# nglaze00/SCoNe_GCN

Measured on NVIDIA B200. Metric: SCoNe train trajectories/sec, higher is better.
Workload: dtype f32

## Files before the change

include/scone_b200.h:

```cpp
#ifndef SCONE_B200_H
#define SCONE_B200_H

#include <stdint.h>

#ifdef __cplusplus
extern "C" {
#endif

#define SCONE_B200_VERSION 100

typedef struct scone_complex scone_complex;
typedef struct scone_model scone_model;

enum { SCONE_MODEL_SCONE = 0, SCONE_MODEL_EBLI = 1, SCONE_MODEL_BUNCH = 2 };
enum { SCONE_ACT_TANH = 0, SCONE_ACT_LEAKY_RELU = 1, SCONE_ACT_RELU = 2 };

int scone_version(void);
const char* scone_last_error(void);

int scone_complex_create(int32_t n_nodes, int32_t n_edges, int32_t n_tris,
                         const int32_t* edge_nodes , const int8_t* edge_signs ,
                         const int32_t* tri_edges , const int8_t* tri_signs ,
                         int32_t model, scone_complex** out);
int scone_complex_create_index_only(int32_t n_nodes, int32_t n_edges, int32_t n_tris,
                                    const int32_t* edge_nodes, const int8_t* edge_signs,
                                    const int32_t* tri_edges, const int8_t* tri_signs,
                                    int32_t model, scone_complex** out);
int scone_complex_destroy(scone_complex* cx);
int scone_complex_dims(const scone_complex* cx, int32_t* n_nodes, int32_t* n_edges, int32_t* n_tris,
                       int32_t* max_degree, int64_t* nnz0, int64_t* nnz1);
int scone_complex_get_shift_csr(const scone_complex* cx, int32_t which, int32_t* rowptr ,
                                int32_t* col , float* val );
int scone_complex_get_nbrhoods(const scone_complex* cx, int32_t* nbrhoods );
int scone_complex_get_edge_rank(const scone_complex* cx, int32_t* rank );


int scone_flows_to_dense(const scone_complex* cx, int32_t b, const int32_t* traj_ptr_dev ,
                         const int32_t* flow_edge_dev, const float* flow_val_dev, float* X_dev ,
                         uint8_t* occ_X_dev , void* stream);

int64_t scone_occ_scratch_bytes(const scone_complex* cx, int32_t b);
int scone_layer_forward(const scone_complex* cx, int32_t act, int32_t b, int32_t cin, int32_t cout,
                        const float* Hin_dev, const float* W0_dev, const float* W1_dev, const float* W2_dev,
                        float* Hout_dev, const uint8_t* occ_in_dev, uint8_t* occ_out_dev, uint8_t* occ_scratch_dev,
                        void* stream);

int64_t scone_layer_backward_workspace_bytes(int32_t cin, int32_t cout);
int scone_layer_backward(const scone_complex* cx, int32_t act, int32_t b, int32_t cin, int32_t cout,
                         const float* G_dev, const float* Hin_dev,
                         const float* W0_dev, const float* W1_dev, const float* W2_dev,
                         float* Gprev_dev, float* dW_dev, int32_t accumulate, void* workspace_dev,
                         const uint8_t* occ_g_dev, const uint8_t* occ_hin_dev, uint8_t* occ_gprev_dev,
                         uint8_t* occ_scratch_dev, void* stream);

int64_t scone_readout_workspace(int32_t b, int32_t C);
int scone_readout(const scone_complex* cx, int32_t act, int32_t b, int32_t C,
                  const float* HL_dev, const float* wout_dev, const int32_t* last_nodes_dev,
                  float* logprobs_dev,
                  const int32_t* target_idx_dev, const float* mask_dev, float scale,
                  float* GL_dev, float* dwout_dev, float* nll_sum_dev, float* count_dev, int32_t accumulate,
                  void* workspace_dev, const uint8_t* occ_HL_dev, uint8_t* occ_GL_dev, void* stream);

int scone_model_create(const scone_complex* cx, int32_t n_layers, const int32_t* hidden, int32_t micro_batch,
                       scone_model** out);
int scone_model_destroy(scone_model* m);
int64_t scone_model_num_params(const scone_model* m);
int scone_model_set_zero_fill(scone_model* m, int32_t on);
int scone_model_get_zero_fill(const scone_model* m);
int scone_model_set_pipeline(scone_model* m, int32_t which);
int scone_model_get_pipeline(const scone_model* m);
int scone_model_set_weights(scone_model* m, const float* weights_host);
int scone_model_get_weights(const scone_model* m, float* weights_host);
float* scone_model_weights_dev(scone_model* m);
float* scone_model_grads_dev(scone_model* m);

int scone_model_forward_host(scone_model* m, int32_t B, const int32_t* traj_ptr ,
                             const int32_t* flow_edge, const float* flow_val, const int32_t* last_nodes,
                             float* logprobs_out , void* stream);
int scone_model_forward_dev(scone_model* m, int32_t B, const int32_t* traj_ptr_dev, const int32_t* flow_edge_dev,
                            const float* flow_val_dev, const int32_t* last_nodes_dev, float* logprobs_dev, void* stream);

int scone_model_loss_grad_dev(scone_model* m, int32_t B, const int32_t* traj_ptr_dev, const int32_t* flow_edge_dev,
                              const float* flow_val_dev, const int32_t* last_nodes_dev,
                              const int32_t* target_idx_dev, const float* mask_dev, int32_t zero_first, void* stream);
int scone_model_loss_grad_host(scone_model* m, int32_t B, const int32_t* traj_ptr, const int32_t* flow_edge,
                               const float* flow_val, const int32_t* last_nodes,
                               const int32_t* target_idx, const float* mask, int32_t zero_first, void* stream);
int scone_accuracy_dev(int32_t B, int32_t D, const float* logprobs_dev, const int32_t* n_nbrs_dev,
                       const int32_t* target_idx_dev, const float* mask_dev, int32_t* out_dev , void* stream);
int scone_model_accuracy_host(scone_model* m, int32_t B, const int32_t* traj_ptr, const int32_t* flow_edge,
                              const float* flow_val, const int32_t* last_nodes, const int32_t* n_nbrs,
                              const int32_t* target_idx, const float* mask, int32_t* out_host , void* stream);
int scone_model_eval_host(scone_model* m, int32_t B, const int32_t* traj_ptr, const int32_t* flow_edge, const float* flow_val,
                          const int32_t* last_nodes, const int32_t* n_nbrs, const int32_t* target_idx, const float* mask,
                          int32_t* choice_out, int32_t* acc_out, float* nll_out, void* stream);
int scone_model_two_target_host(scone_model* m, int32_t B, const int32_t* true_idx, const int32_t* rand_idx, int32_t* out ,
                                void* stream);
int scone_model_read_grads(scone_model* m, float* out_host, void* stream);
int scone_model_read_grads_async(scone_model* m, float* out_pinned, void* stream);

int scone_model_adam_step(scone_model* m, int32_t step, float lr, float weight_decay, void* stream);

typedef struct scone_dp scone_dp;
int scone_dp_create(int32_t rank, int32_t world, int64_t n_floats, scone_dp** out);
int32_t scone_dp_handle_bytes(void);
int scone_dp_get_handle(scone_dp* dp, void* handle_out);
int scone_dp_open(scone_dp* dp, const void* handles_rank_major);
int scone_model_dp_adam_step(scone_model* m, scone_dp* dp, int32_t step, float lr, float wd, void* stream);
int scone_dp_status(scone_dp* dp, void* stream);
void scone_dp_destroy(scone_dp* dp);
int scone_model_plan_host(scone_model* m, int32_t B, const int32_t* traj_ptr, const int32_t* flow_edge, const float* flow_val,
                          const int32_t* last_nodes, void* stream);
int scone_model_plan_dev(scone_model* m, int32_t B, const int32_t* traj_ptr_dev, const int32_t* flow_edge_dev, const float* flow_val_dev,
                         const int32_t* last_nodes_dev, void* stream);
int scone_model_loss_grad_planned_host(scone_model* m, int32_t n, const int32_t* rows, const int32_t* target_idx, const float* mask,
                                       int32_t zero_first, void* stream);
int scone_model_loss_grad_planned_dev(scone_model* m, int32_t n, const int32_t* rows_dev, const int32_t* target_idx_dev, const float* mask_dev,
                                      int32_t zero_first, void* stream);
int scone_model_forward_planned_host(scone_model* m, int32_t n, const int32_t* rows, float* logprobs_out , void* stream);
int scone_model_check_overflow(scone_model* m, void* stream);
int scone_model_set_weights_keep_state(scone_model* m, const float* weights_host, void* stream);
int scone_model_fused_info(const scone_model* m, int32_t* out );
int scone_model_fused_read(scone_model* m, int32_t t, int32_t* hdr_out , uint32_t off, int32_t words, uint32_t* arena_out);
int scone_model_read_rows_done(scone_model* m, int64_t* out );

typedef struct scone_csr scone_csr;
typedef struct scone_bunch scone_bunch;
int scone_csr_create(int32_t rows, int32_t cols, const int32_t* rowptr , const int32_t* col, const float* val,
                     scone_csr** out);
int scone_csr_destroy(scone_csr* S);
int scone_bunch_create(const scone_csr* const* S7, int32_t n_nodes, int32_t n_edges, int32_t n_tris, int32_t max_degree,
                       const int32_t* nbrhoods , int32_t n_hidden, const int32_t* hidden,
                       int32_t micro_batch, scone_bunch** out);
int scone_bunch_destroy(scone_bunch* m);
int64_t scone_bunch_num_params(const scone_bunch* m);
float* scone_bunch_grads_dev(scone_bunch* m);
int scone_bunch_set_weights(scone_bunch* m, const float* weights_host, int32_t reset_adam);
int scone_bunch_get_weights(const scone_bunch* m, float* weights_host);
int scone_bunch_forward_host(scone_bunch* m, int32_t B, const int32_t* traj_ptr, const int32_t* flow_edge, const float* flow_val,
                             const int32_t* last_nodes, float* logprobs_out , void* stream);
int scone_bunch_loss_grad_host(scone_bunch* m, int32_t B, const int32_t* traj_ptr, const int32_t* flow_edge, const float* flow_val,
                               const int32_t* last_nodes, const int32_t* target_idx, const float* mask, int32_t zero_first,
                               void* stream);
int scone_bunch_read_grads(scone_bunch* m, float* out_host, void* stream);
int scone_bunch_adam_step(scone_bunch* m, int32_t step, float lr, float weight_decay, void* stream);

int scone_set_zero_fill(int32_t on);
int scone_get_zero_fill(void);

int scone_set_dense_kernel(int32_t which);
int scone_umma_status(void* stream);
int scone_set_dense_chunk(int32_t tiles);
int scone_get_dense_kernel(void);

int scone_profile_enable(int32_t on);
int scone_profile_reset(void);
int scone_profile_read(int32_t kind, int64_t* launches, double* total_ms);
int scone_profile_read_rows(int32_t kind, int64_t* rows);

int64_t scone_launch_count(void);

#ifdef __cplusplus
}
#endif
#endif
```

scone_gcn_b200/_lib.py:

```python
import ctypes as C
import os

_HERE = os.path.dirname(os.path.abspath(__file__))
_LIB = None


class LibraryMissing(RuntimeError):
    pass


class SconeError(RuntimeError):
    pass


def library_path():
    return os.path.join(_HERE, 'libscone_b200.so')


_i32, _i64, _f32, _vp = C.c_int32, C.c_int64, C.c_float, C.c_void_p
DEFAULT_DENSE_KERNEL = 3

SIGNATURES = {
    'scone_version': (C.c_int, []),
    'scone_last_error': (C.c_char_p, []),
    'scone_launch_count': (_i64, []),
    'scone_profile_enable': (C.c_int, [_i32]),
    'scone_profile_reset': (C.c_int, []),
    'scone_profile_read': (C.c_int, [_i32, C.POINTER(_i64), C.POINTER(C.c_double)]),
    'scone_profile_read_rows': (C.c_int, [_i32, C.POINTER(_i64)]),
    'scone_complex_create': (C.c_int, [_i32, _i32, _i32, _vp, _vp, _vp, _vp, _i32, C.POINTER(_vp)]),
    'scone_complex_create_index_only': (C.c_int, [_i32, _i32, _i32, _vp, _vp, _vp, _vp, _i32, C.POINTER(_vp)]),
    'scone_complex_destroy': (C.c_int, [_vp]),
    'scone_complex_dims': (C.c_int, [_vp] + [C.POINTER(_i32)] * 4 + [C.POINTER(_i64)] * 2),
    'scone_complex_get_shift_csr': (C.c_int, [_vp, _i32, _vp, _vp, _vp]),
    'scone_complex_get_nbrhoods': (C.c_int, [_vp, _vp]),
    'scone_complex_get_edge_rank': (C.c_int, [_vp, _vp]),
    'scone_flows_to_dense': (C.c_int, [_vp, _i32, _vp, _vp, _vp, _vp, _vp, _vp]),
    'scone_occ_scratch_bytes': (_i64, [_vp, _i32]),
    'scone_layer_forward': (C.c_int, [_vp, _i32, _i32, _i32, _i32, _vp, _vp, _vp, _vp, _vp, _vp, _vp, _vp, _vp]),
    'scone_layer_backward_workspace_bytes': (_i64, [_i32, _i32]),
    'scone_layer_backward': (C.c_int, [_vp, _i32, _i32, _i32, _i32, _vp, _vp, _vp, _vp, _vp, _vp, _vp, _i32, _vp, _vp, _vp, _vp, _vp, _vp]),
    'scone_readout_workspace': (_i64, [_i32, _i32]),
    'scone_readout': (C.c_int, [_vp, _i32, _i32, _i32, _vp, _vp, _vp, _vp, _vp, _vp, _f32, _vp, _vp, _vp, _vp, _i32, _vp, _vp, _vp, _vp]),
    'scone_set_zero_fill': (C.c_int, [_i32]),
    'scone_get_zero_fill': (C.c_int, []),
    'scone_set_dense_kernel': (C.c_int, [_i32]),
    'scone_set_dense_chunk': (C.c_int, [_i32]),
    'scone_get_dense_kernel': (C.c_int, []),
    'scone_umma_status': (C.c_int, [_vp]),
    'scone_csr_create': (C.c_int, [_i32, _i32, _vp, _vp, _vp, C.POINTER(_vp)]),
    'scone_csr_destroy': (C.c_int, [_vp]),
    'scone_bunch_create': (C.c_int, [_vp, _i32, _i32, _i32, _i32, _vp, _i32, _vp, _i32, C.POINTER(_vp)]),
    'scone_bunch_destroy': (C.c_int, [_vp]),
    'scone_bunch_num_params': (_i64, [_vp]),
    'scone_bunch_grads_dev': (_vp, [_vp]),
    'scone_bunch_set_weights': (C.c_int, [_vp, _vp, _i32]),
    'scone_bunch_get_weights': (C.c_int, [_vp, _vp]),
    'scone_bunch_forward_host': (C.c_int, [_vp, _i32, _vp, _vp, _vp, _vp, _vp, _vp]),
    'scone_bunch_loss_grad_host': (C.c_int, [_vp, _i32, _vp, _vp, _vp, _vp, _vp, _vp, _i32, _vp]),
    'scone_bunch_read_grads': (C.c_int, [_vp, _vp, _vp]),
    'scone_bunch_adam_step': (C.c_int, [_vp, _i32, _f32, _f32, _vp]),
    'scone_model_create': (C.c_int, [_vp, _i32, _vp, _i32, C.POINTER(_vp)]),
    'scone_model_destroy': (C.c_int, [_vp]),
    'scone_model_num_params': (_i64, [_vp]),
    'scone_model_set_zero_fill': (C.c_int, [_vp, _i32]),
    'scone_model_get_zero_fill': (C.c_int, [_vp]),
    'scone_model_set_pipeline': (C.c_int, [_vp, _i32]),
    'scone_model_get_pipeline': (C.c_int, [_vp]),
    'scone_model_set_weights': (C.c_int, [_vp, _vp]),
    'scone_model_get_weights': (C.c_int, [_vp, _vp]),
    'scone_model_weights_dev': (_vp, [_vp]),
    'scone_model_grads_dev': (_vp, [_vp]),
    'scone_model_forward_host': (C.c_int, [_vp, _i32, _vp, _vp, _vp, _vp, _vp, _vp]),
    'scone_model_forward_dev': (C.c_int, [_vp, _i32, _vp, _vp, _vp, _vp, _vp, _vp]),
    'scone_model_loss_grad_dev': (C.c_int, [_vp, _i32, _vp, _vp, _vp, _vp, _vp, _vp, _i32, _vp]),
    'scone_model_loss_grad_host': (C.c_int, [_vp, _i32, _vp, _vp, _vp, _vp, _vp, _vp, _i32, _vp]),
    'scone_accuracy_dev': (C.c_int, [_i32, _i32, _vp, _vp, _vp, _vp, _vp, _vp]),
    'scone_model_accuracy_host': (C.c_int, [_vp, _i32, _vp, _vp, _vp, _vp, _vp, _vp, _vp, _vp, _vp]),
    'scone_model_read_grads': (C.c_int, [_vp, _vp, _vp]),
    'scone_model_read_grads_async': (C.c_int, [_vp, _vp, _vp]),
    'scone_model_eval_host': (C.c_int, [_vp, _i32] + [_vp] * 10 + [_vp]),
    'scone_model_two_target_host': (C.c_int, [_vp, _i32, _vp, _vp, _vp, _vp]),
    'scone_model_adam_step': (C.c_int, [_vp, _i32, _f32, _f32, _vp]),
    'scone_dp_create': (C.c_int, [_i32, _i32, _i64, C.POINTER(_vp)]),
    'scone_dp_handle_bytes': (_i32, []),
    'scone_dp_get_handle': (C.c_int, [_vp, _vp]),
    'scone_dp_open': (C.c_int, [_vp, _vp]),
    'scone_model_dp_adam_step': (C.c_int, [_vp, _vp, _i32, _f32, _f32, _vp]),
    'scone_dp_status': (C.c_int, [_vp, _vp]),
    'scone_dp_destroy': (None, [_vp]),
    'scone_model_check_overflow': (C.c_int, [_vp, _vp]),
    'scone_model_plan_host': (C.c_int, [_vp, _i32, _vp, _vp, _vp, _vp, _vp]),
    'scone_model_plan_dev': (C.c_int, [_vp, _i32, _vp, _vp, _vp, _vp, _vp]),
    'scone_model_loss_grad_planned_host': (C.c_int, [_vp, _i32, _vp, _vp, _vp, _i32, _vp]),
    'scone_model_loss_grad_planned_dev': (C.c_int, [_vp, _i32, _vp, _vp, _vp, _i32, _vp]),
    'scone_model_forward_planned_host': (C.c_int, [_vp, _i32, _vp, _vp, _vp]),
    'scone_model_set_weights_keep_state': (C.c_int, [_vp, _vp, _vp]),
    'scone_model_fused_info': (C.c_int, [_vp, _vp]),
    'scone_model_fused_read': (C.c_int, [_vp, _i32, _vp, C.c_uint32, _i32, _vp]),
    'scone_model_read_rows_done': (C.c_int, [_vp, _vp]),
}


def lib():
    global _LIB
    if _LIB is not None:
        return _LIB
    path = library_path()
    if not os.path.exists(path):
        raise LibraryMissing(
            '%s not found: build it with `python __graft_entry__.py build` (or `make`). '
            'scone_gcn_b200 has no CPU fallback.' % path)
    L = C.CDLL(path)
    for name, (res, args) in SIGNATURES.items():
        f = getattr(L, name)
        f.restype, f.argtypes = res, args
    _LIB = L
    return L


def check(rc, what=''):
    if rc != 0:
        msg = lib().scone_last_error().decode('utf-8', 'replace')
        raise SconeError('%s failed (code %d): %s' % (what or 'scone call', rc, msg))


def ptr(a):
    if a is None:
        return None
    assert a.flags['C_CONTIGUOUS']
    return a.ctypes.data_as(C.c_void_p)


def dptr(t):
    if t is None:
        return None
    if isinstance(t, int):
        return C.c_void_p(t)
    assert t.is_cuda and t.is_contiguous()
    return C.c_void_p(t.data_ptr())
```

scone_gcn_b200/csrc/fused.cuh:

```cuda
#pragma once
#include "common.cuh"

constexpr int kFusedMaxL = 3;
constexpr int kFusedHdrW = 16;
constexpr int kFusedFlagOverflow = 1;
constexpr int kFusedFlagRetry = 2;

struct PlanArgs {
    const int32_t* traj_ptr;
    const int32_t* flow_edge;
    const float* flow_val;
    const int32_t* last_nodes;
    const int32_t* rank;
    const int32_t* nbrhoods;
    const int32_t* inc_ptr;
    const int2* inc_ent;
    const int32_t* mptr;
    const int2* ment;
    int N, D, E, L;
    int HS, hshift;
    const unsigned* cone_ptr;
    const uint32_t* cone_ent;
    int LV;
    int EC;
    int M;
    const unsigned long long* node_off;
    const unsigned* tb_rowptr;
    const int2* tb_ent;
    const unsigned* pair_ptr;
    const int2* tb_pairs;
    const int* pair_off;
    int* hdr;
    uint32_t* arena;
    unsigned long long* bump;
    unsigned long long arena_words;
    int* overflow;
    int tier;
    int n_work;
    int t0;
    const int* n_in;
    const int* in_list;
    int* n_retry;
    int* retry;
};

#ifdef __CUDACC__
template <int THREADS>
__device__ inline int fused_block_scan_excl(int* a, int n, int* s_warp) {
    const int tid = threadIdx.x, lane = tid & 31, warp = tid >> 5;
    const int per = (n + THREADS - 1) / THREADS;
    const int lo = min(n, tid * per), hi = min(n, lo + per);
    int sum = 0;
    for (int i = lo; i < hi; ++i) sum += a[i];
    int inc = sum;
#pragma unroll
    for (int o = 1; o < 32; o <<= 1) {
        const int v = __shfl_up_sync(0xffffffffu, inc, o);
        if (lane >= o) inc += v;
    }
    __syncthreads();
    if (lane == 31) s_warp[warp] = inc;
    __syncthreads();
    int base = 0, total = 0;
#pragma unroll
    for (int w = 0; w < THREADS / 32; ++w) {
        const int v = s_warp[w];
        if (w < warp) base += v;
        total += v;
    }
    int run = base + inc - sum;
    for (int i = lo; i < hi; ++i) {
        const int v = a[i];
        a[i] = run;
        run += v;
    }
    if (tid == 0) a[n] = total;
    __syncthreads();
    return total;
}
#endif

struct FusedState {
    int L = 0, C = 0;
    int64_t n_params = 0;
    int bound_cone = 0, bound_list = 0;
    unsigned* d_cone_ptr = nullptr;
    uint32_t* d_cone_ent = nullptr;
    unsigned long long cone_entries = 0;
    bool tb_rows = false;
    unsigned long long* d_node_off = nullptr;
    unsigned* d_tb_rowptr = nullptr;
    int2* d_tb_ent = nullptr;
    unsigned* d_pair_ptr = nullptr;
    int2* d_tb_pairs = nullptr;
    int* d_pair_off = nullptr;
    unsigned long long tb_entries = 0, tb_bytes = 0;
    int tbM0 = 0, tbLV0 = 0, tbM1 = 0, tbLV1 = 0, tbM = 0, tbLV = 0;
    size_t tb_smem0 = 0, tb_smem1 = 0, tb_smem = 0;
    bool tb_two_tiers = false, tb_mid_tier = false;
    int quantile_cone = 0;
    int HS = 0, LV = 0, EC = 0, hshift = 0;
    int HS0 = 0, LV0 = 0, EC0 = 0, hshift0 = 0;
    bool two_tiers = false;
    int flow_room = 0;
    size_t plan_smem0 = 0;
    unsigned long long worst_words = 0;
    int* d_retry = nullptr;
    size_t plan_smem = 0, traj_smem_small = 0, traj_smem_big = 0;
    int cap_rows = 0, big_rows = 0, grid_small = 0, grid_big = 0, chunk = 0;
    size_t scratch_stride = 0;
    unsigned long long arena_words = 0;
    int* d_hdr = nullptr;
    uint32_t* d_arena = nullptr;
    unsigned long long* d_bump = nullptr;
    float* d_partial = nullptr;
    float* d_scratch = nullptr;
    int* d_stats = nullptr;
    unsigned long long* d_rows_done = nullptr;
    uint32_t* d_sort = nullptr;
    void* d_sort_tmp = nullptr;
    size_t sort_tmp_bytes = 0;
    int sort_cap = 0;
    int* d_set_hdr = nullptr;
    uint32_t* d_set_arena = nullptr;
    unsigned long long* d_set_bump = nullptr;
    unsigned long long set_arena_words = 0;
    int set_cap = 0, set_n = 0;
};

int scone_table_build(const scone_complex* cx, FusedState* f, int L, bool* ok);
int scone_table_plan_launch(const FusedState* f, PlanArgs p, int b, int num_sms, cudaStream_t st, int phase = 2);
void scone_table_destroy(FusedState* f);

bool scone_fused_supported(const scone_complex* cx, int n_layers, const int32_t* hidden);
int scone_fused_create(const scone_complex* cx, int L, int C, int mb, int64_t n_params, FusedState** out);
void scone_fused_destroy(FusedState* f);
int scone_fused_run(const scone_complex* cx, FusedState* f, int act, int b, const int32_t* traj_ptr, const int32_t* flow_edge,
                    const float* flow_val, const int32_t* last_nodes, const float* W, const int64_t* w_off, float* logprobs,
                    const int32_t* target_idx, const float* mask, float* grad, int* overflow, bool count_rows, cudaStream_t st);
int scone_fused_begin(FusedState* f, cudaStream_t st);
int scone_fused_plan_part(const scone_complex* cx, FusedState* f, int off, int b, const int32_t* traj_ptr, const int32_t* flow_edge,
                          const float* flow_val, const int32_t* last_nodes, int* overflow, cudaStream_t st,
                          bool defer_tiers = false);
int scone_fused_plan_finish(const scone_complex* cx, FusedState* f, int B, const int32_t* traj_ptr, const int32_t* flow_edge,
                            const float* flow_val, const int32_t* last_nodes, int* overflow, cudaStream_t st);
int scone_fused_compute(const scone_complex* cx, FusedState* f, int act, int b, const float* W, const int64_t* w_off, float* logprobs,
                        const int32_t* target_idx, const float* mask, float* grad, bool count_rows, cudaStream_t st);
int scone_fused_plan_set(const scone_complex* cx, FusedState* f, int B, const int32_t* traj_ptr, const int32_t* flow_edge,
                         const float* flow_val, const int32_t* last_nodes, int* overflow, cudaStream_t st);
int scone_fused_run_planned(const scone_complex* cx, FusedState* f, int act, int n, const int32_t* rows_dev, const float* W, const int64_t* w_off,
                            float* logprobs, const int32_t* target_idx, const float* mask, float* grad, bool count_rows, cudaStream_t st);
int scone_fused_last_retries(FusedState* f);
int scone_fused_read(FusedState* f, int t, int* hdr_out, unsigned off, int words, uint32_t* arena_out);
```

scone_gcn_b200/csrc/scone_fused.cu:

```cuda
#include <algorithm>
#include <cstdlib>
#include <cub/device/device_radix_sort.cuh>
#include "common.cuh"
#include "fused.cuh"

namespace {

#include "slab_common.cuh"

constexpr int kTrajThreads = 256;
constexpr int kFuMaxD = 128;
constexpr uint32_t kNoRow = 0xFFFFu;
constexpr uint32_t kFlaggedKey = 0xFFFFFFu;

template <int ACT>
__device__ __forceinline__ float fu_act(float z) {
    if (ACT == SCONE_ACT_TANH) return scone_tanh(z);
    if (ACT == SCONE_ACT_LEAKY_RELU) return z >= 0.f ? z : 0.01f * z;
    return fmaxf(z, 0.f);
}
template <int ACT>
__device__ __forceinline__ float fu_dact(float h) {
    if (ACT == SCONE_ACT_TANH) return 1.f - h * h;
    if (ACT == SCONE_ACT_LEAKY_RELU) return h >= 0.f ? 1.f : 0.01f;
// ... 825 lines not shown
                }
                fu_dw<C>(acc[l - 2], hprev + (size_t)r0 * G::LDH, tile, nr);
                __syncthreads();
                fu_product<C, true>(tile, Wl, nr, [&](int r, int col, float v0, float v1) {
                    const float2 hv = *reinterpret_cast<const float2*>(hprev + (size_t)(r0 + r) * G::LDH + col);
                    *reinterpret_cast<float2*>(gprev + (size_t)(r0 + r) * G::LDH + col) =
                        make_float2(v0 * fu_dact<ACT>(hv.x), v1 * fu_dact<ACT>(hv.y));
                });
                cp_async_wait_all();
                __syncthreads();
                r0 += nr;
            }
            if (np_ == 0) {
                cp_async_wait_all();
                __syncthreads();
            }
            pf = pf_next;
        }
        if (tid < 3 * C) {
            const int k = tid / C, c = tid % C;
            const float* g1 = rows;
            float s = acc1;
            for (int r = 0; r < n[1]; ++r) s = fmaf(l1[3 * r + k], g1[(size_t)r * G::LDH + c], s);
            acc1 = s;
        }
        if (have_next && !issued_next) {
            cp_async_wait_all();
            __syncthreads();
            pf_first_next = issue_first(s_hdr[(k + 1) & 1], l1s + ((k + 1) & 1) * G::SL1);
        }
        pf_first = pf_first_next;
        t = t_next;
        have = have_next;
    }

    if (a.rows_done != nullptr && tid == 0 && (n_fwd | n_bwd)) {
        atomicAdd(a.rows_done, n_fwd);
        atomicAdd(a.rows_done + 1, n_bwd);
    }
    if (!GRAD) return;
    float* P = a.partial + (size_t)blockIdx.x * (a.n_params + 2);
    if (tid < 3 * C) P[a.w_off[tid / C] + tid % C] = acc1;
    {
        const int g = lane >> 2, tig = lane & 3;
        const int mt = warp % G::NMT, ntg = warp / G::NMT;
#pragma unroll
        for (int l = 2; l <= kFusedMaxL; ++l) {
            if (l > L) break;
#pragma unroll
            for (int s = 0; s < G::TPW; ++s) {
                const int nt = ntg + G::WPM * s;
                if (nt >= G::NNT) continue;
                const int nn = 8 * nt + 2 * tig, term = nn / C, co = nn % C;
                float* dst = P + a.w_off[3 * (l - 1) + term];
                const int ci = 16 * mt + g;
                dst[ci * C + co] = acc[l - 2][s][0];
                dst[ci * C + co + 1] = acc[l - 2][s][1];
                dst[(ci + 8) * C + co] = acc[l - 2][s][2];
                dst[(ci + 8) * C + co + 1] = acc[l - 2][s][3];
            }
        }
    }
    if (tid < C) P[a.w_off[3 * L] + tid] = acc_out;
    if (warp == 0) {
        float s = acc_nll;
#pragma unroll
        for (int o = 16; o > 0; o >>= 1) s += __shfl_xor_sync(0xffffffffu, s, o);
        if (lane == 0) {
            P[a.n_params] = s;
            P[a.n_params + 1] = acc_cnt;
        }
    }
}

__global__ void __launch_bounds__(256) fused_cost_kernel(const int* __restrict__ hdr, const int32_t* __restrict__ rows, int b, int L,
                                                         uint32_t* __restrict__ keys, int32_t* __restrict__ vals) {
    const int t = blockIdx.x * blockDim.x + threadIdx.x;
    if (t >= b) return;
    const int* h = hdr + (size_t)(rows != nullptr ? rows[t] : t) * kFusedHdrW;
    int tot = 0;
    for (int l = 1; l <= L; ++l) tot += h[l];
    keys[t] = h[0] != 0 ? kFlaggedKey : min((uint32_t)tot, kFlaggedKey - 1u);
    vals[t] = t;
}

__global__ void __launch_bounds__(256) fused_reduce_kernel(const float* __restrict__ partial, int nparts, int n, float* __restrict__ out) {
    __shared__ float red[8][32];
    const int lane = threadIdx.x & 31, warp = threadIdx.x >> 5;
    const int i = blockIdx.x * 32 + lane;
    float s = 0.f;
    if (i < n)
        for (int p = warp; p < nparts; p += 8) s += partial[(size_t)p * n + i];
    red[warp][lane] = s;
    __syncthreads();
    if (warp == 0 && i < n)
        out[i] += ((red[0][lane] + red[1][lane]) + (red[2][lane] + red[3][lane])) + ((red[4][lane] + red[5][lane]) + (red[6][lane] + red[7][lane]));
}

size_t plan_smem_bytes(int HS, int LV, int EC) {
    return (size_t)HS * 18 + (size_t)(LV + 4) * 8 + (size_t)LV * 10 + (size_t)EC * 2 + 16;
}

template <int C>
size_t traj_smem_bytes(int D, int cap_rows) {
    using G = FuGeom<C>;
    size_t fl = (size_t)(kFusedMaxL - 1) * 3 * C * G::LDW + 3 * C + C + (size_t)G::CH * G::LDA + (size_t)D * C + 2 * ((D + 3) & ~3) +
                2 * (size_t)G::SE + G::SP + 2 * G::SL1 + (size_t)cap_rows * G::LDH;
    return fl * sizeof(float);
}

template <int C, int ACT, bool GRAD>
int launch_traj(const TrajArgs& base, int grid_small, int grid_big, size_t smem_small, size_t smem_big, cudaStream_t st) {
    static bool configured = false;
    if (!configured) {
        SCONE_CUDA(cudaFuncSetAttribute(fused_traj_kernel<C, ACT, GRAD, false>, cudaFuncAttributeMaxDynamicSharedMemorySize, 227 * 1024 - 1024));
        SCONE_CUDA(cudaFuncSetAttribute(fused_traj_kernel<C, ACT, GRAD, true>, cudaFuncAttributeMaxDynamicSharedMemorySize, 227 * 1024 - 1024));
        configured = true;
    }
    TrajArgs a = base;
    fused_traj_kernel<C, ACT, GRAD, false><<<grid_small, kTrajThreads, smem_small, st>>>(a);
    SCONE_LAUNCHED();
    if (grid_big > 0) {
        if (GRAD) a.partial = base.partial + (size_t)grid_small * (base.n_params + 2);
        fused_traj_kernel<C, ACT, GRAD, true><<<grid_big, kTrajThreads, smem_big, st>>>(a);
        SCONE_LAUNCHED();
    }
    return 0;
}

template <int C, bool GRAD>
int dispatch_traj(int act, const TrajArgs& a, int gs, int gb, size_t ss, size_t sb, cudaStream_t st) {
    switch (act) {
        case SCONE_ACT_TANH: return launch_traj<C, SCONE_ACT_TANH, GRAD>(a, gs, gb, ss, sb, st);
        case SCONE_ACT_LEAKY_RELU: return launch_traj<C, SCONE_ACT_LEAKY_RELU, GRAD>(a, gs, gb, ss, sb, st);
        case SCONE_ACT_RELU: return launch_traj<C, SCONE_ACT_RELU, GRAD>(a, gs, gb, ss, sb, st);
    }
    scone_set_error("unknown activation %d", act);
    return 2;
}

int run_traj(FusedState* f, int act, TrajArgs& t, float* grad, cudaStream_t st) {
    const bool want_grad = grad != nullptr;
    const int n = t.b;
    if (n > f->sort_cap) {
        cudaFree(f->d_sort);
        cudaFree(f->d_sort_tmp);
        f->d_sort = nullptr;
        f->d_sort_tmp = nullptr;
        f->sort_cap = 0;
        uint32_t* k = nullptr;
        int32_t* v = nullptr;
        size_t bytes = 0;
        SCONE_CUDA(cub::DeviceRadixSort::SortPairsDescending(nullptr, bytes, k, k, v, v, n, 0, 24, st));
        SCONE_CUDA(cudaMalloc((void**)&f->d_sort, 4 * (size_t)n * sizeof(uint32_t)));
        SCONE_CUDA(cudaMalloc((void**)&f->d_sort_tmp, bytes ? bytes : 16));
        f->sort_tmp_bytes = bytes;
        f->sort_cap = n;
    }
    uint32_t* k_in = f->d_sort;
    uint32_t* k_out = k_in + f->sort_cap;
    int32_t* v_in = reinterpret_cast<int32_t*>(k_out + f->sort_cap);
    int32_t* v_out = v_in + f->sort_cap;
    ScopedProf prof(want_grad ? SCONE_K_LAYER_BWD : SCONE_K_LAYER_FWD, st);
    fused_cost_kernel<<<(n + 255) / 256, 256, 0, st>>>(t.hdr, t.rows, n, f->L, k_in, v_in);
    SCONE_LAUNCHED();
    size_t bytes = f->sort_tmp_bytes;
    SCONE_CUDA(cub::DeviceRadixSort::SortPairsDescending(f->d_sort_tmp, bytes, k_in, k_out, v_in, v_out, n, 0, 24, st));
    t.okeys = k_out;
    t.order = v_out;
    int rc;
    if (f->C == 32)
        rc = want_grad ? dispatch_traj<32, true>(act, t, f->grid_small, f->grid_big, f->traj_smem_small, f->traj_smem_big, st)
                       : dispatch_traj<32, false>(act, t, f->grid_small, f->grid_big, f->traj_smem_small, f->traj_smem_big, st);
    else
        rc = want_grad ? dispatch_traj<16, true>(act, t, f->grid_small, f->grid_big, f->traj_smem_small, f->traj_smem_big, st)
                       : dispatch_traj<16, false>(act, t, f->grid_small, f->grid_big, f->traj_smem_small, f->traj_smem_big, st);
    if (rc) return rc;
    if (want_grad) {
        const int np = (int)f->n_params + 2;
        fused_reduce_kernel<<<(np + 31) / 32, 256, 0, st>>>(f->d_partial, f->grid_small + f->grid_big, np, grad);
        SCONE_LAUNCHED();
    }
    return 0;
}

}

bool scone_fused_supported(const scone_complex* cx, int n_layers, const int32_t* hidden) {
    if (cx->d_mptr == nullptr || cx->D > kFuMaxD || cx->D < 1 || n_layers < 1 || n_layers > kFusedMaxL) return false;
    for (int l = 0; l < n_layers; ++l)
        if (hidden[l] != hidden[0] || (hidden[l] != 16 && hidden[l] != 32)) return false;
    return true;
}

void scone_fused_destroy(FusedState* f) {
    if (!f) return;
    cudaFree(f->d_hdr); cudaFree(f->d_retry); cudaFree(f->d_arena); cudaFree(f->d_set_hdr); cudaFree(f->d_set_arena); cudaFree(f->d_set_bump); cudaFree(f->d_bump); cudaFree(f->d_partial); cudaFree(f->d_scratch); cudaFree(f->d_stats);
    cudaFree(f->d_rows_done); cudaFree(f->d_sort); cudaFree(f->d_sort_tmp);
    scone_table_destroy(f);
    delete f;
}

static void table_shape(int entries, int* HS, int* hshift) {
    int hs = 256;
    while (hs * 3 / 4 < entries + 1) hs *= 2;
    *HS = hs;
    *hshift = 32;
    for (int v = hs; v > 1; v >>= 1) --*hshift;
}

int scone_fused_create(const scone_complex* cx, int L, int C, int mb, int64_t n_params, FusedState** out) {
    *out = nullptr;
    if ((unsigned)cx->E >= (1u << 30)) return 0;
    FusedState* f = new FusedState();
    f->L = L;
    f->C = C;
    f->n_params = n_params;
    {
        bool ok = false;
        const int rc = scone_table_build(cx, f, L, &ok);
        if (rc || !ok) {
            scone_fused_destroy(f);
            return rc;
        }
    }
    int max_row = 1;
    {
        std::vector<int32_t> mp((size_t)cx->E + 1);
        SCONE_CUDA(cudaMemcpy(mp.data(), cx->d_mptr, mp.size() * sizeof(int32_t), cudaMemcpyDeviceToHost));
        for (int e = 0; e < cx->E; ++e) max_row = std::max(max_row, mp[e + 1] - mp[e]);
    }
    constexpr int kMaxPlanSmem = 225 * 1024;
    f->LV = (f->bound_list + 63) & ~63;
    table_shape(f->bound_cone, &f->HS, &f->hshift);
    f->EC = (int)std::min<long long>((long long)f->bound_list * max_row, 1ll << 30);
    f->EC = (f->EC + 63) & ~63;
    {
        const size_t fixed = plan_smem_bytes(f->HS, f->LV, 0);
        if (fixed + 2 * (size_t)f->EC > (size_t)kMaxPlanSmem && fixed + 2 * 8192 <= (size_t)kMaxPlanSmem)
            f->EC = (int)(((size_t)kMaxPlanSmem - fixed) / 2) & ~63;
    }
    f->plan_smem = plan_smem_bytes(f->HS, f->LV, f->EC);
    if (!f->tb_rows && (f->plan_smem > (size_t)kMaxPlanSmem || f->bound_list >= 0xFFFF || f->HS > 32768)) {
        scone_fused_destroy(f);
        return 0;
    }
    {
        table_shape(f->quantile_cone, &f->HS0, &f->hshift0);
        f->LV0 = std::min(192, f->LV);
        f->EC0 = std::min(3072, f->EC);
        f->two_tiers = f->HS0 < f->HS || f->LV0 < f->LV || f->EC0 < f->EC;
        if (!f->two_tiers) {
            f->HS0 = f->HS;
            f->hshift0 = f->hshift;
        }
        auto env_int = [](const char* name, int dflt) {
            const char* v = getenv(name);
            return v && *v ? atoi(v) : dflt;
        };
        if (f->two_tiers) {
            const int hs0 = env_int("SCONE_FUSED_HS0", f->HS0);
            if (hs0 != f->HS0 && hs0 >= 256 && hs0 <= f->HS && (hs0 & (hs0 - 1)) == 0) table_shape((hs0 * 3) / 4 - 1, &f->HS0, &f->hshift0);
            f->LV0 = std::min(env_int("SCONE_FUSED_LV0", f->LV0), f->LV);
            f->EC0 = std::min(env_int("SCONE_FUSED_EC0", f->EC0), f->EC);
        }
        f->plan_smem0 = plan_smem_bytes(f->HS0, f->LV0, f->EC0);
    }
    SCONE_CUDA(cudaFuncSetAttribute(fused_plan_kernel<256>, cudaFuncAttributeMaxDynamicSharedMemorySize, kMaxPlanSmem));
    SCONE_CUDA(cudaFuncSetAttribute(fused_plan_kernel<1024>, cudaFuncAttributeMaxDynamicSharedMemorySize, kMaxPlanSmem));
    const int ldh = C + 8;
    f->cap_rows = C == 32 ? 192 : 384;
    f->big_rows = L * f->bound_list;
    f->traj_smem_small = C == 32 ? traj_smem_bytes<32>(cx->D, f->cap_rows) : traj_smem_bytes<16>(cx->D, f->cap_rows);
    f->traj_smem_big = C == 32 ? traj_smem_bytes<32>(cx->D, 0) : traj_smem_bytes<16>(cx->D, 0);
    if (f->traj_smem_small > 113 * 1024) {
        const size_t over = f->traj_smem_small - 113 * 1024;
        const int less = (int)((over + ldh * 4 - 1) / (ldh * 4));
        f->cap_rows = f->cap_rows > less + 32 ? f->cap_rows - less : 32;
        f->traj_smem_small = C == 32 ? traj_smem_bytes<32>(cx->D, f->cap_rows) : traj_smem_bytes<16>(cx->D, f->cap_rows);
    }
    f->grid_small = 2 * cx->num_sms;
    f->grid_big = f->big_rows > f->cap_rows ? 2 * cx->num_sms : 0;
    if (f->grid_big) {
        f->scratch_stride = (size_t)f->big_rows * ldh;
        SCONE_CUDA(cudaMalloc((void**)&f->d_scratch, (size_t)f->grid_big * f->scratch_stride * sizeof(float)));
    }
    SCONE_CUDA(cudaMalloc((void**)&f->d_partial, (size_t)(f->grid_small + f->grid_big) * (n_params + 2) * sizeof(float)));
    const unsigned long long bl = (unsigned long long)f->bound_list;
    unsigned long long worst = 3 * bl + 2 + (unsigned long long)(cx->D + 3) + 2ull * cx->D * cx->D + 16;
    for (int l = 2; l <= L; ++l)
        worst += 2 * (bl + 3) + 4 * bl * (unsigned long long)max_row;
    const unsigned long long budget_words = (1ull << 30) - 1024;
    const unsigned long long share_words = 16 * 1024;
    f->worst_words = worst;
    if (worst * (unsigned long long)mb <= budget_words) {
        f->chunk = mb;
        f->arena_words = worst * (unsigned long long)mb;
    } else {
        f->chunk = (int)std::min<unsigned long long>((unsigned long long)mb, std::max<unsigned long long>(1, budget_words / std::min(worst, share_words)));
        f->arena_words = std::min(budget_words, worst * (unsigned long long)f->chunk);
    }
    SCONE_CUDA(cudaMalloc((void**)&f->d_arena, f->arena_words * sizeof(uint32_t)));
    SCONE_CUDA(cudaMalloc((void**)&f->d_hdr, (size_t)f->chunk * kFusedHdrW * sizeof(int)));
    SCONE_CUDA(cudaMalloc((void**)&f->d_retry, 2 * (size_t)f->chunk * sizeof(int)));
    SCONE_CUDA(cudaMalloc((void**)&f->d_bump, 2 * sizeof(unsigned long long)));
    SCONE_CUDA(cudaMalloc((void**)&f->d_rows_done, 4 * sizeof(unsigned long long)));
    SCONE_CUDA(cudaMemset(f->d_rows_done, 0, 4 * sizeof(unsigned long long)));
    *out = f;
    return 0;
}

static int launch_plans(const scone_complex* cx, const FusedState* f, PlanArgs p, int b, cudaStream_t st) {
    if (f->tb_rows) return scone_table_plan_launch(f, p, b, cx->num_sms, st);
    p.tier = 0; p.n_work = b;
    p.HS = f->HS0; p.LV = f->LV0; p.EC = f->EC0; p.hshift = f->hshift0;
    int* retry = p.retry;
    if (!f->two_tiers) p.retry = nullptr;
    fused_plan_kernel<256><<<b, 256, f->plan_smem0, st>>>(p);
    SCONE_LAUNCHED();
    if (f->two_tiers) {
        p.tier = 1; p.HS = f->HS; p.LV = f->LV; p.EC = f->EC; p.hshift = f->hshift; p.n_in = p.n_retry; p.in_list = retry; p.retry = nullptr;
        fused_plan_kernel<1024><<<std::min(b, cx->num_sms), 1024, f->plan_smem, st>>>(p);
        SCONE_LAUNCHED();
    }
    return 0;
}

int scone_fused_begin(FusedState* f, cudaStream_t st) {
    SCONE_CUDA(cudaMemsetAsync(f->d_bump, 0, 2 * sizeof(unsigned long long), st));
    return 0;
}

static PlanArgs plan_args(const scone_complex* cx, FusedState* f, int off, const int32_t* traj_ptr, const int32_t* flow_edge,
                          const float* flow_val, const int32_t* last_nodes, int* overflow) {
    PlanArgs p{};
    p.traj_ptr = traj_ptr + off; p.flow_edge = flow_edge; p.flow_val = flow_val; p.last_nodes = last_nodes + off;
    p.rank = cx->d_rank; p.nbrhoods = cx->d_nbrhoods; p.inc_ptr = cx->d_inc_ptr; p.inc_ent = cx->d_inc_ent;
    p.mptr = cx->d_mptr; p.ment = cx->d_ment; p.cone_ptr = f->d_cone_ptr; p.cone_ent = f->d_cone_ent;
    p.N = cx->N; p.D = cx->D; p.E = cx->E; p.L = f->L;
    p.hdr = f->d_hdr + (size_t)off * kFusedHdrW; p.arena = f->d_arena; p.bump = f->d_bump; p.arena_words = f->arena_words; p.overflow = overflow;
    p.n_retry = reinterpret_cast<int*>(f->d_bump + 1); p.retry = f->d_retry;
    return p;
}

int scone_fused_plan_part(const scone_complex* cx, FusedState* f, int off, int b, const int32_t* traj_ptr, const int32_t* flow_edge,
                          const float* flow_val, const int32_t* last_nodes, int* overflow, cudaStream_t st, bool defer_tiers) {
    if (b <= 0) return 0;
    SCONE_REQUIRE(off >= 0 && off + b <= f->chunk, "scone_fused_plan_part: trajectories %d .. %d exceed the planned chunk of %d", off, off + b, f->chunk);
    ScopedProf prof(SCONE_K_CONE, st);
    if (defer_tiers && f->tb_rows) {
        PlanArgs p = plan_args(cx, f, 0, traj_ptr, flow_edge, flow_val, last_nodes, overflow);
        p.t0 = off;
        return scone_table_plan_launch(f, p, b, cx->num_sms, st, 0);
    }
    if (off > 0) SCONE_CUDA(cudaMemsetAsync(f->d_bump + 1, 0, sizeof(unsigned long long), st));
    return launch_plans(cx, f, plan_args(cx, f, off, traj_ptr, flow_edge, flow_val, last_nodes, overflow), b, st);
}

int scone_fused_plan_finish(const scone_complex* cx, FusedState* f, int B, const int32_t* traj_ptr, const int32_t* flow_edge,
                            const float* flow_val, const int32_t* last_nodes, int* overflow, cudaStream_t st) {
    if (B <= 0 || !f->tb_rows) return 0;
    ScopedProf prof(SCONE_K_CONE, st);
    return scone_table_plan_launch(f, plan_args(cx, f, 0, traj_ptr, flow_edge, flow_val, last_nodes, overflow), B, cx->num_sms, st, 1);
}

int scone_fused_compute(const scone_complex* cx, FusedState* f, int act, int b, const float* W, const int64_t* w_off, float* logprobs,
                        const int32_t* target_idx, const float* mask, float* grad, bool count_rows, cudaStream_t st) {
    if (b <= 0) return 0;
    TrajArgs t;
    t.hdr = f->d_hdr; t.arena = f->d_arena; t.rows = nullptr; t.W = W;
    for (int i = 0; i <= 3 * kFusedMaxL; ++i) t.w_off[i] = i <= 3 * f->L ? (int)w_off[i] : 0;
    t.L = f->L; t.b = b; t.D = cx->D; t.n_params = (int)f->n_params;
    t.logprobs = logprobs; t.target_idx = target_idx; t.mask = mask;
    t.partial = f->d_partial; t.scratch = f->d_scratch; t.scratch_stride = f->scratch_stride;
    t.cap_rows = f->cap_rows; t.big_rows = f->big_rows;
    t.rows_done = count_rows ? f->d_rows_done : nullptr;
    return run_traj(f, act, t, grad, st);
}

int scone_fused_run(const scone_complex* cx, FusedState* f, int act, int b, const int32_t* traj_ptr, const int32_t* flow_edge,
                    const float* flow_val, const int32_t* last_nodes, const float* W, const int64_t* w_off, float* logprobs,
                    const int32_t* target_idx, const float* mask, float* grad, int* overflow, bool count_rows, cudaStream_t st) {
    if (b <= 0) return 0;
    SCONE_REQUIRE(b <= f->chunk, "scone_fused_run: chunk of %d trajectories exceeds the planned %d", b, f->chunk);
    int rc = scone_fused_begin(f, st);
    if (!rc) rc = scone_fused_plan_part(cx, f, 0, b, traj_ptr, flow_edge, flow_val, last_nodes, overflow, st);
    if (!rc) rc = scone_fused_compute(cx, f, act, b, W, w_off, logprobs, target_idx, mask, grad, count_rows, st);
    return rc;
}

int scone_fused_plan_set(const scone_complex* cx, FusedState* f, int B, const int32_t* traj_ptr, const int32_t* flow_edge,
                         const float* flow_val, const int32_t* last_nodes, int* overflow, cudaStream_t st) {
    if (B > f->set_cap) {
        cudaFree(f->d_set_hdr);
        cudaFree(f->d_set_arena);
        f->d_set_hdr = nullptr;
        f->d_set_arena = nullptr;
        f->set_cap = 0;
        const unsigned long long budget_words = (1ull << 30) - 1024;
        f->set_arena_words = std::min(budget_words, f->worst_words * (unsigned long long)B);
        SCONE_CUDA(cudaMalloc((void**)&f->d_set_hdr, (size_t)B * kFusedHdrW * sizeof(int)));
        SCONE_CUDA(cudaMalloc((void**)&f->d_set_arena, f->set_arena_words * sizeof(uint32_t)));
        if (!f->d_set_bump) SCONE_CUDA(cudaMalloc((void**)&f->d_set_bump, 2 * sizeof(unsigned long long)));
        f->set_cap = B;
    }
    f->set_n = 0;
    SCONE_CUDA(cudaMemsetAsync(f->d_set_bump, 0, 2 * sizeof(unsigned long long), st));
    PlanArgs p{};
    p.flow_edge = flow_edge; p.flow_val = flow_val;
    p.rank = cx->d_rank; p.nbrhoods = cx->d_nbrhoods; p.inc_ptr = cx->d_inc_ptr; p.inc_ent = cx->d_inc_ent;
    p.mptr = cx->d_mptr; p.ment = cx->d_ment; p.cone_ptr = f->d_cone_ptr; p.cone_ent = f->d_cone_ent;
    p.N = cx->N; p.D = cx->D; p.E = cx->E; p.L = f->L;
    p.arena = f->d_set_arena; p.bump = f->d_set_bump; p.arena_words = f->set_arena_words; p.overflow = overflow;
    p.n_retry = reinterpret_cast<int*>(f->d_set_bump + 1); p.retry = f->d_retry;
    ScopedProf prof(SCONE_K_CONE, st);
    for (int off = 0; off < B; off += f->chunk) {
        const int b = std::min(f->chunk, B - off);
        SCONE_CUDA(cudaMemsetAsync(f->d_set_bump + 1, 0, sizeof(unsigned long long), st));
        p.traj_ptr = traj_ptr + off; p.last_nodes = last_nodes + off; p.hdr = f->d_set_hdr + (size_t)off * kFusedHdrW;
        const int rc = launch_plans(cx, f, p, b, st);
        if (rc) return rc;
    }
    f->set_n = B;
    return 0;
}

int scone_fused_run_planned(const scone_complex* cx, FusedState* f, int act, int n, const int32_t* rows_dev, const float* W, const int64_t* w_off,
                            float* logprobs, const int32_t* target_idx, const float* mask, float* grad, bool count_rows, cudaStream_t st) {
    if (n <= 0) return 0;
    SCONE_REQUIRE(f->set_n > 0, "scone_fused_run_planned: no planned set (call scone_model_plan_* first)");
    SCONE_REQUIRE(rows_dev != nullptr || n <= f->set_n, "scone_fused_run_planned: %d trajectories requested, the planned set holds %d", n, f->set_n);
    TrajArgs t;
    t.hdr = f->d_set_hdr; t.arena = f->d_set_arena; t.rows = rows_dev; t.W = W;
    for (int i = 0; i <= 3 * kFusedMaxL; ++i) t.w_off[i] = i <= 3 * f->L ? (int)w_off[i] : 0;
    t.L = f->L; t.b = n; t.D = cx->D; t.n_params = (int)f->n_params;
    t.logprobs = logprobs; t.target_idx = target_idx; t.mask = mask;
    t.partial = f->d_partial; t.scratch = f->d_scratch; t.scratch_stride = f->scratch_stride;
    t.cap_rows = f->cap_rows; t.big_rows = f->big_rows;
    t.rows_done = count_rows ? f->d_rows_done : nullptr;
    return run_traj(f, act, t, grad, st);
}

int scone_fused_last_retries(FusedState* f) {
    unsigned long long v[2] = {0, 0};
    if (cudaDeviceSynchronize() != cudaSuccess) return -1;
    if (cudaMemcpy(v, f->d_bump, sizeof(v), cudaMemcpyDeviceToHost) != cudaSuccess) return -1;
    return (int)(v[1] & 0xffffffffull);
}

int scone_fused_read(FusedState* f, int t, int* hdr_out, unsigned off, int words, uint32_t* arena_out) {
    SCONE_CUDA(cudaDeviceSynchronize());
    if (hdr_out) SCONE_CUDA(cudaMemcpy(hdr_out, f->d_hdr + (size_t)t * kFusedHdrW, kFusedHdrW * sizeof(int), cudaMemcpyDeviceToHost));
    if (arena_out && words > 0) SCONE_CUDA(cudaMemcpy(arena_out, f->d_arena + off, (size_t)words * sizeof(uint32_t), cudaMemcpyDeviceToHost));
    return 0;
}
```

scone_gcn_b200/csrc/scone_model.cu:

```cuda
#include <algorithm>
#include <cstring>
#include "common.cuh"
#include "fused.cuh"

struct scone_model {
    const scone_complex* cx = nullptr;
    int32_t L = 0, mb = 0, act = 0, cmax = 0;
    std::vector<int32_t> hidden;
    std::vector<int64_t> w_off;
    int64_t n_params = 0;
    float *d_w = nullptr, *d_m = nullptr, *d_v = nullptr, *d_grad = nullptr;
    float* d_X = nullptr;
    std::vector<float*> d_H;
    std::vector<float*> d_G;
    std::vector<uint8_t*> d_occH;
    std::vector<uint8_t*> d_occG;
    cudaStream_t side = nullptr;
    cudaStream_t compute = nullptr;
    cudaEvent_t ev_fork = nullptr, ev_join = nullptr;
    cudaEvent_t ev_begin = nullptr;
    cudaStream_t copy = nullptr;
    cudaEvent_t ev_copy0 = nullptr, ev_part[8] = {nullptr, nullptr, nullptr, nullptr, nullptr, nullptr, nullptr, nullptr};
    cudaEvent_t ev_plan_done = nullptr;
    long long staging_epoch = 0, plan_done_epoch = -1;
// ... 357 lines not shown
        const int cout = m->hidden[l];
        ScopedProf prof(l == 0 ? SCONE_K_LAYER0_FWD : SCONE_K_LAYER_FWD, s);
        const float *W0 = m->d_w + m->w_off[3 * l], *W1 = m->d_w + m->w_off[3 * l + 1], *W2 = m->d_w + m->w_off[3 * l + 2];
        int rc;
        if (l == 0)
            rc = scone_rows_layer0_forward(cx, m->act, b, cout, m->d_X, W0, W1, W2, m->d_cH[0], m->d_rowsC[0], cone_n(m, 0), nullptr,
                                           m->row_cap, m->d_overflow, s);
        else
            rc = scone_slab_forward_rows(cx, m->act, b, cin, cout, m->d_cH[l - 1], W0, W1, W2, m->d_cH[l], nullptr, m->d_rowsC[l],
                                         cone_n(m, l), scone_prof_row_counter(SCONE_K_LAYER_FWD), m->d_bmGr[l - 1], m->d_prefG[l - 1],
                                         m->row_cap, m->d_overflow, s);
        if (rc) return rc;
        cin = cout;
    }
    return 0;
}

int cone_readout(scone_model* m, int32_t b, const int32_t* last, float* logprobs, bool grad, const int32_t* tgt, const float* mask,
                 cudaStream_t s) {
    const scone_complex* cx = m->cx;
    const int L = m->L, CL = m->hidden[L - 1];
    const float* wout = m->d_w + m->w_off[3 * L];
    ScopedProf prof(SCONE_K_READOUT, s);
    if (scone_rows_readout_forward(cx, b, CL, m->d_cH[L - 1], wout, last, logprobs, m->d_bmGr[L - 1], m->d_prefG[L - 1], nullptr, nullptr, s))
        return 1;
    if (!grad) return 0;
    return scone_rows_readout_backward(cx, m->act, b, CL, m->d_cH[L - 1], wout, last, logprobs, tgt, mask, 1.f, m->d_cG[L - 1],
                                       cone_n(m, L - 1), m->row_cap, m->d_overflow, m->d_grad + m->w_off[3 * L], m->d_grad + m->n_params,
                                       m->d_grad + m->n_params + 1, 1, (float*)m->d_ws, m->d_bmGr[L - 1], m->d_prefG[L - 1],
                                       m->d_bmGr[L - 1], m->d_prefG[L - 1], s);
}

int cone_backward_mb(scone_model* m, int32_t b, cudaStream_t s) {
    const scone_complex* cx = m->cx;
    const int L = m->L;
    const int a_cap = m->row_cap < m->a_cap ? m->row_cap : m->a_cap;
    SCONE_CUDA(cudaMemset2DAsync(m->d_nrows + 1, 2 * sizeof(int), 0, sizeof(int), (size_t)(L + 1), s));
    for (int l = L - 1; l >= 1; --l) {
        ScopedProf prof(SCONE_K_LAYER_BWD, s);
        int rc = scone_rows_backward(cx, m->act, b, m->hidden[l - 1], m->hidden[l], m->d_cG[l], m->d_cH[l - 1], m->d_cG[l - 1], m->d_Abuf,
                                     m->d_w + m->w_off[3 * l], m->d_w + m->w_off[3 * l + 1], m->d_w + m->w_off[3 * l + 2], m->d_rowsC[l - 1],
                                     cone_n(m, l - 1), m->d_bmGr[l], m->d_bmGr[l - 1], a_cap, m->d_overflow, m->d_grad + m->w_off[3 * l], 1,
                                     (float*)m->d_ws, m->d_prefG[l], m->d_prefG[l - 1], true, s);
        if (rc) return rc;
    }
    ScopedProf prof(SCONE_K_LAYER0_BWD, s);
    return scone_rows_layer0_backward(cx, b, m->hidden[0], m->d_X, m->d_cG[0], m->d_rowsC[0], cone_n(m, 0), m->d_grad + m->w_off[0], 1,
                                      (float*)m->d_ws, m->row_cap, s);
}

}

extern "C" int scone_model_create(const scone_complex* cx, int32_t n_layers, const int32_t* hidden, int32_t micro_batch,
                                  scone_model** out) {
    SCONE_REQUIRE(out != nullptr, "scone_model_create: out is NULL");
    *out = nullptr;
    SCONE_REQUIRE(cx && hidden && n_layers >= 1 && micro_batch >= 1, "scone_model_create: bad arguments");
    SCONE_REQUIRE(!cx->host_only, "scone_model_create: index-only complex has no device arrays");
    scone_model* m = new scone_model();
    m->cx = cx;
    m->L = n_layers;
    m->mb = micro_batch;
    m->act = cx->model == SCONE_MODEL_EBLI ? SCONE_ACT_LEAKY_RELU : SCONE_ACT_TANH;
    m->hidden.assign(hidden, hidden + n_layers);
    int64_t off = 0;
    int cin = 1;
    for (int l = 0; l < n_layers; ++l) {
        const int c = hidden[l];
        if (!(c == 8 || c == 16 || c == 32 || c == 64)) {
            scone_set_error("scone_model_create: hidden width %d of layer %d unsupported (8, 16, 32 or 64)", c, l);
            delete m;
            return 2;
        }
        if (l > 0 && !(c == cin || c == 2 * cin || 2 * c == cin)) {
            scone_set_error("scone_model_create: consecutive widths %d -> %d unsupported (ratio must be 1/2, 1 or 2)", cin, c);
            delete m;
            return 2;
        }
        for (int k = 0; k < 3; ++k) {
            m->w_off.push_back(off);
            off += (int64_t)cin * c;
        }
        m->cmax = c > m->cmax ? c : m->cmax;
        cin = c;
    }
    m->w_off.push_back(off);
    off += cin;
    m->n_params = off;
    const size_t E = cx->E, mb = micro_batch;
    int rc = 0;
    auto alloc = [&](void** p, size_t bytes) {
        if (rc) return;
        cudaError_t e = cudaMalloc(p, bytes ? bytes : 4);
        if (e != cudaSuccess) {
            scone_set_error("scone_model_create: cudaMalloc(%zu bytes) failed: %s", bytes, cudaGetErrorString(e));
            rc = 1;
        }
    };
    alloc((void**)&m->d_w, off * sizeof(float));
    alloc((void**)&m->d_m, off * sizeof(float));
    alloc((void**)&m->d_v, off * sizeof(float));
    alloc((void**)&m->d_grad, (off + 2) * sizeof(float));
    m->d_H.assign(n_layers, nullptr);
    m->d_G.assign(n_layers, nullptr);
    m->d_occH.assign(n_layers, nullptr);
    m->d_occG.assign(n_layers, nullptr);
    m->rows_ok = scone_rows_supported(cx, n_layers, hidden) && E * mb < ((size_t)1 << 32);
    m->pipeline = m->rows_ok ? ((cx->D <= 32 || E * mb >= ((size_t)1 << 31)) ? 3 : 2) : 0;
    if (scone_fused_supported(cx, n_layers, hidden)) {
        if (scone_fused_create(cx, n_layers, hidden[0], micro_batch, m->n_params, &m->fused)) {
            delete m;
            return 1;
        }
        if (m->fused) m->pipeline = 4;
    }
    if (m->pipeline != 4 && !m->rows_ok && E * mb >= ((size_t)1 << 31)) {
        scone_set_error("scone_model_create: E * micro_batch = %zu needs the row-list pipeline (widths 16 / 32, E * micro_batch < 2^32)", E * mb);
        delete m;
        return 2;
    }
    int64_t ws = scone_readout_workspace_bytes(micro_batch, m->cmax);
    if (scone_rows_dw_workspace_bytes(m->cmax, m->cmax) > ws) ws = scone_rows_dw_workspace_bytes(m->cmax, m->cmax);
    cin = 1;
    for (int l = 0; l < n_layers; ++l) {
        int64_t w = scone_layer_backward_workspace_bytes(cin, hidden[l]);
        ws = w > ws ? w : ws;
        cin = hidden[l];
    }
    alloc(&m->d_ws, ws);
    alloc((void**)&m->d_logp, mb * (size_t)(cx->D > 0 ? cx->D : 1) * sizeof(float));
    if (!rc) {
        int prio_lo = 0, prio_hi = 0;
        cudaDeviceGetStreamPriorityRange(&prio_lo, &prio_hi);
        cudaStreamCreateWithPriority(&m->side, cudaStreamNonBlocking, prio_lo);
        cudaStreamCreateWithPriority(&m->compute, cudaStreamNonBlocking, prio_hi);
        cudaEventCreateWithFlags(&m->ev_fork, cudaEventDisableTiming);
        cudaEventCreateWithFlags(&m->ev_join, cudaEventDisableTiming);
        cudaEventCreateWithFlags(&m->ev_begin, cudaEventDisableTiming);
        m->ev_fill.assign(2 * n_layers, nullptr);
        for (auto& e : m->ev_fill) cudaEventCreateWithFlags(&e, cudaEventDisableTiming);
        cudaMemset(m->d_w, 0, off * sizeof(float));
        cudaMemset(m->d_m, 0, off * sizeof(float));
        cudaMemset(m->d_v, 0, off * sizeof(float));
        cudaMemset(m->d_grad, 0, (off + 2) * sizeof(float));
    }
    if (!rc) rc = ensure_buffers(m);
    if (rc) {
        scone_model_destroy(m);
        return rc;
    }
    *out = m;
    return 0;
}

extern "C" int scone_model_destroy(scone_model* m) {
    if (!m) return 0;
    cudaFree(m->d_w); cudaFree(m->d_m); cudaFree(m->d_v); cudaFree(m->d_grad); cudaFree(m->d_X);
    for (float* p : m->d_H) cudaFree(p);
    for (uint8_t* p : m->d_occH) cudaFree(p);
    for (uint8_t* p : m->d_occG) cudaFree(p);
    cudaFree(m->d_occS); cudaFree(m->d_occX); cudaFree(m->d_bmX); cudaFree(m->d_bmG);
    for (uint32_t* p : m->d_bmH) cudaFree(p);
    for (uint32_t* p : m->d_bmGr) cudaFree(p);
    for (uint32_t* p : m->d_prefH) cudaFree(p);
    for (uint32_t* p : m->d_prefG) cudaFree(p);
    for (float* p : m->d_cH) cudaFree(p);
    for (float* p : m->d_cG) cudaFree(p);
    for (uint32_t* p : m->d_rowsC) cudaFree(p);
    for (uint32_t* p : m->d_bmC) cudaFree(p);
    cudaFree(m->d_rows); cudaFree(m->d_nrows); cudaFree(m->d_overflow); cudaFree(m->d_tickets); cudaFree(m->d_Abuf);
    for (float* p : m->d_G) cudaFree(p);
    cudaFree(m->d_ws); cudaFree(m->d_logp);
    scone_fused_destroy(m->fused);
    if (m->side) cudaStreamDestroy(m->side);
    if (m->compute) cudaStreamDestroy(m->compute);
    if (m->ev_fork) cudaEventDestroy(m->ev_fork);
    if (m->ev_join) cudaEventDestroy(m->ev_join);
    if (m->ev_begin) cudaEventDestroy(m->ev_begin);
    if (m->copy) cudaStreamDestroy(m->copy);
    if (m->ev_copy0) cudaEventDestroy(m->ev_copy0);
    if (m->ev_plan_done) cudaEventDestroy(m->ev_plan_done);
    for (auto e : m->ev_part) if (e) cudaEventDestroy(e);
    for (auto e : m->ev_fill) if (e) cudaEventDestroy(e);
    cudaFree(m->d_ptr); cudaFree(m->d_edge); cudaFree(m->d_last); cudaFree(m->d_tgt); cudaFree(m->d_val);
    cudaFree(m->d_mask); cudaFree(m->d_logp_all); cudaFree(m->d_nn); cudaFree(m->d_acc);
    cudaFree(m->d_choice); cudaFree(m->d_rand); cudaFree(m->d_evalf);
    delete m;
    return 0;
}

extern "C" int64_t scone_model_num_params(const scone_model* m) { return m ? m->n_params : -1; }
extern "C" int scone_model_set_zero_fill(scone_model* m, int32_t on) {
    SCONE_REQUIRE(m != nullptr, "scone_model_set_zero_fill: NULL model");
    SCONE_REQUIRE(!on || (size_t)m->cx->E * m->mb < ((size_t)1 << 31), "scone_model_set_zero_fill: E * micro_batch >= 2^31 runs on pipeline 3 only");
    m->zero_fill = on != 0;
    return ensure_buffers(m);
}
extern "C" int scone_model_get_zero_fill(const scone_model* m) { return m && m->zero_fill ? 1 : 0; }
extern "C" int scone_model_set_pipeline(scone_model* m, int32_t which) {
    SCONE_REQUIRE(m != nullptr && which >= 0 && which <= 4,
                  "scone_model_set_pipeline: 0 (unit kernels, byte flags), 1 (row lists, dense tensors), 2 (row lists, compact tensors), "
                  "3 (compact row lists over the readout cone) or 4 (trajectory-fused kernels)");
    SCONE_REQUIRE(which != 4 || m->fused != nullptr,
                  "scone_model_set_pipeline: the fused pipeline needs one uniform hidden width of 16 or 32, at most 3 layers, and cones that fit "
                  "its shared-memory tables");
    SCONE_REQUIRE(which == 0 || which == 4 || m->rows_ok, "scone_model_set_pipeline: the row-list pipelines need hidden widths in {16, 32}");
    SCONE_REQUIRE(which >= 3 || (size_t)m->cx->E * m->mb < ((size_t)1 << 31),
                  "scone_model_set_pipeline: E * micro_batch >= 2^31 runs on pipelines 3 / 4 only");
    SCONE_REQUIRE(which != 3 || (size_t)m->cx->E * m->mb < ((size_t)1 << 32), "scone_model_set_pipeline: pipeline 3 needs E * micro_batch < 2^32");
    const int old = m->pipeline;
    m->pipeline = which;
    if (ensure_buffers(m)) {
        m->pipeline = old;
        return 1;
    }
    return 0;
}
extern "C" int scone_model_get_pipeline(const scone_model* m) { return m ? (m->zero_fill ? 0 : m->pipeline) : -1; }
extern "C" float* scone_model_weights_dev(scone_model* m) { return m ? m->d_w : nullptr; }
extern "C" float* scone_model_grads_dev(scone_model* m) { return m ? m->d_grad : nullptr; }

extern "C" int scone_model_set_weights(scone_model* m, const float* w) {
    SCONE_REQUIRE(m && w, "scone_model_set_weights: NULL argument");
    SCONE_CUDA(cudaMemcpy(m->d_w, w, m->n_params * sizeof(float), cudaMemcpyHostToDevice));
    SCONE_CUDA(cudaMemset(m->d_m, 0, m->n_params * sizeof(float)));
    SCONE_CUDA(cudaMemset(m->d_v, 0, m->n_params * sizeof(float)));
    return 0;
}

extern "C" int scone_model_get_weights(const scone_model* m, float* w) {
    SCONE_REQUIRE(m && w, "scone_model_get_weights: NULL argument");
    SCONE_CUDA(cudaMemcpy(w, m->d_w, m->n_params * sizeof(float), cudaMemcpyDeviceToHost));
    return 0;
}

static int fork_to_compute(scone_model* m, void* user_st) {
    SCONE_CUDA(cudaEventRecord(m->ev_fork, as_stream(user_st)));
    SCONE_CUDA(cudaStreamWaitEvent(m->compute, m->ev_fork, 0));
    return 0;
}
static int join_from_compute(scone_model* m, void* user_st) {
    SCONE_CUDA(cudaEventRecord(m->ev_join, m->compute));
    SCONE_CUDA(cudaStreamWaitEvent(as_stream(user_st), m->ev_join, 0));
    return 0;
}

static int finish_call(scone_model* m, int rc, void* user_st) {
    if (rc) {
        m->x_clean = false;
        m->cone_clean = false;
    }
    const int jr = join_from_compute(m, user_st);
    return rc ? rc : jr;
}

static int fused_call(scone_model* m, int32_t B, const int32_t* ptr, const int32_t* edge, const float* val, const int32_t* last,
                      float* logprobs, const int32_t* tgt, const float* mask, bool grad, cudaStream_t s) {
    const int step = m->fused->chunk < m->mb ? m->fused->chunk : m->mb;
    for (int32_t off = 0; off < B; off += step) {
        const int32_t b = B - off < step ? B - off : step;
        int rc = scone_fused_run(m->cx, m->fused, m->act, b, ptr + off, edge, val, last + off, m->d_w, m->w_off.data(),
                                 logprobs ? logprobs + (size_t)off * m->cx->D : nullptr, grad ? tgt + off : nullptr,
                                 grad ? mask + off : nullptr, grad ? m->d_grad : nullptr, m->d_overflow, g_scone_prof, s);
        if (rc) return rc;
    }
    return 0;
}

static bool fused_host_overlap_ok(const scone_model* m, int32_t B, int64_t nnz) {
    const bool rows = m->pipeline >= 1 && !m->zero_fill;
    return rows && m->pipeline == 4 && m->fused && B >= 512 && B <= m->fused->chunk && B <= m->mb && nnz >= (1 << 13);
}

static int fused_host_overlapped(scone_model* m, int32_t B, const int32_t* ptr, const int32_t* edge, const float* val, float* logprobs_dev,
                                 bool grad, int32_t zero_first, cudaStream_t s) {
    constexpr int kMaxParts = 4;
    const int kParts = B >= 4 * 4096 ? 4 : (B >= 2 * 4096 ? 2 : 1);
    if (!m->copy) {
        SCONE_CUDA(cudaStreamCreateWithFlags(&m->copy, cudaStreamNonBlocking));
        SCONE_CUDA(cudaEventCreateWithFlags(&m->ev_copy0, cudaEventDisableTiming));
        SCONE_CUDA(cudaEventCreateWithFlags(&m->ev_plan_done, cudaEventDisableTiming));
        for (auto& e : m->ev_part) SCONE_CUDA(cudaEventCreateWithFlags(&e, cudaEventDisableTiming));
    }
    if (m->plan_done_epoch >= 0 && m->plan_done_epoch == m->staging_epoch - 1) {
        SCONE_CUDA(cudaStreamWaitEvent(m->copy, m->ev_plan_done, 0));
    } else {
        SCONE_CUDA(cudaEventRecord(m->ev_copy0, s));
        SCONE_CUDA(cudaStreamWaitEvent(m->copy, m->ev_copy0, 0));
    }
    int32_t b0[kMaxParts + 1];
    for (int k = 0; k <= kParts; ++k) b0[k] = (int32_t)((int64_t)B * k / kParts);
    for (int k = 0; k < kParts; ++k) {
        const int64_t q0 = ptr[b0[k]], q1 = ptr[b0[k + 1]];
        if (q1 > q0) {
            SCONE_CUDA(cudaMemcpyAsync(m->d_edge + q0, edge + q0, (q1 - q0) * sizeof(int32_t), cudaMemcpyHostToDevice, m->copy));
            SCONE_CUDA(cudaMemcpyAsync(m->d_val + q0, val + q0, (q1 - q0) * sizeof(float), cudaMemcpyHostToDevice, m->copy));
        }
        SCONE_CUDA(cudaEventRecord(m->ev_part[k], m->copy));
    }
    if (fork_to_compute(m, (void*)s)) return 1;
    cudaStream_t c = m->compute;
    if (grad && zero_first) SCONE_CUDA(cudaMemsetAsync(m->d_grad, 0, (m->n_params + 2) * sizeof(float), c));
    int rc = scone_fused_begin(m->fused, c);
    for (int k = 0; k < kParts && !rc; ++k) {
        SCONE_CUDA(cudaStreamWaitEvent(c, m->ev_part[k], 0));
        rc = scone_fused_plan_part(m->cx, m->fused, b0[k], b0[k + 1] - b0[k], m->d_ptr, m->d_edge, m->d_val, m->d_last, m->d_overflow, c,
                                   kParts > 1);
    }
    if (!rc && kParts > 1) rc = scone_fused_plan_finish(m->cx, m->fused, B, m->d_ptr, m->d_edge, m->d_val, m->d_last, m->d_overflow, c);
    if (!rc) {
        SCONE_CUDA(cudaEventRecord(m->ev_plan_done, c));
        m->plan_done_epoch = m->staging_epoch;
    } else {
        m->plan_done_epoch = -1;
    }
    if (!rc)
        rc = scone_fused_compute(m->cx, m->fused, m->act, B, m->d_w, m->w_off.data(), logprobs_dev, grad ? m->d_tgt : nullptr,
                                 grad ? m->d_mask : nullptr, grad ? m->d_grad : nullptr, g_scone_prof, c);
    return finish_call(m, rc, (void*)s);
}

extern "C" int scone_model_forward_dev(scone_model* m, int32_t B, const int32_t* ptr, const int32_t* edge, const float* val,
                                       const int32_t* last, float* logprobs, void* user_st) {
    SCONE_REQUIRE(m && ptr && last && logprobs && B >= 0, "scone_model_forward_dev: bad arguments");
    if (fork_to_compute(m, user_st)) return 1;
    void* st = (void*)m->compute;
    const scone_complex* cx = m->cx;
    const bool rows = m->pipeline >= 1 && !m->zero_fill;
    if (rows && m->pipeline == 4) return finish_call(m, fused_call(m, B, ptr, edge, val, last, logprobs, nullptr, nullptr, false, as_stream(st)), user_st);
    int rc = 0;
    for (int32_t off = 0; off < B && !rc; off += m->mb) {
        const int32_t b = B - off < m->mb ? B - off : m->mb;
        if (rows && m->pipeline == 3) {
            rc = cone_build_mb(m, b, ptr + off, edge, val, last + off, as_stream(st));
            if (!rc) rc = cone_forward_mb(m, b, as_stream(st));
            if (!rc) rc = cone_readout(m, b, last + off, logprobs + (size_t)off * cx->D, false, nullptr, nullptr, as_stream(st));
            if (!rc) rc = rows_clear_x(m, b, ptr + off, edge, val, as_stream(st));
            if (!rc) rc = cone_clear_mb(m, b, as_stream(st));
            continue;
        }
        if (rows) {
            rc = rows_forward_mb(m, b, ptr + off, edge, val, as_stream(st));
            if (!rc) rc = rows_readout(m, b, last + off, logprobs + (size_t)off * cx->D, false, nullptr, nullptr, as_stream(st));
            if (!rc) rc = rows_clear_x(m, b, ptr + off, edge, val, as_stream(st));
            continue;
        }
        m->x_clean = false;
        rc = start_fills(m, b, false, as_stream(st));
        if (!rc) rc = forward_mb(m, b, ptr + off, edge, val, st);
        if (!rc)
            rc = scone_readout_ws(cx, m->act, b, m->hidden[m->L - 1], m->d_H[m->L - 1], m->d_w + m->w_off[3 * m->L], last + off,
                                  logprobs + (size_t)off * cx->D, nullptr, nullptr, 0.f, nullptr, nullptr, nullptr, nullptr, 0,
                                  nullptr, m->d_occH[m->L - 1], nullptr, st);
    }
    return finish_call(m, rc, user_st);
}

extern "C" int scone_model_loss_grad_dev(scone_model* m, int32_t B, const int32_t* ptr, const int32_t* edge, const float* val,
                                         const int32_t* last, const int32_t* tgt, const float* mask, int32_t zero_first,
                                         void* user_st) {
    SCONE_REQUIRE(m && ptr && last && tgt && mask && B >= 0, "scone_model_loss_grad_dev: bad arguments");
    if (fork_to_compute(m, user_st)) return 1;
    void* st = (void*)m->compute;
    const scone_complex* cx = m->cx;
    const int L = m->L;
    cudaStream_t s = as_stream(st);
    if (zero_first) SCONE_CUDA(cudaMemsetAsync(m->d_grad, 0, (m->n_params + 2) * sizeof(float), s));
    const bool rows = m->pipeline >= 1 && !m->zero_fill;
    if (rows && m->pipeline == 4) return finish_call(m, fused_call(m, B, ptr, edge, val, last, nullptr, tgt, mask, true, s), user_st);
    int rc = 0;
    for (int32_t off = 0; off < B && !rc; off += m->mb) {
        const int32_t b = B - off < m->mb ? B - off : m->mb;
        if (rows && m->pipeline == 3) {
            rc = cone_build_mb(m, b, ptr + off, edge, val, last + off, s);
            if (!rc) rc = cone_forward_mb(m, b, s);
            if (!rc) rc = cone_readout(m, b, last + off, m->d_logp, true, tgt + off, mask + off, s);
            if (!rc) rc = cone_backward_mb(m, b, s);
            if (!rc) rc = rows_clear_x(m, b, ptr + off, edge, val, s);
            if (!rc) rc = cone_clear_mb(m, b, s);
            continue;
        }
        if (rows) {
            rc = rows_forward_mb(m, b, ptr + off, edge, val, s);
            if (!rc) rc = rows_readout(m, b, last + off, m->d_logp, true, tgt + off, mask + off, s);
            if (!rc) rc = rows_backward_mb(m, b, s);
            if (!rc) rc = rows_clear_x(m, b, ptr + off, edge, val, s);
            continue;
        }
        m->x_clean = false;
        rc = start_fills(m, b, true, s);
        if (!rc) rc = forward_mb(m, b, ptr + off, edge, val, st);
        const int CL = m->hidden[L - 1];
        if (!rc && wait_fill(m, L + (L - 1), s)) rc = 1;
        if (rc) break;
        g_scone_hints.out_bm = m->d_bmG;
        rc = scone_readout_ws(cx, m->act, b, CL, m->d_H[L - 1], m->d_w + m->w_off[3 * L], last + off, m->d_logp, tgt + off,
                              mask + off, 1.f, m->d_G[L - 1], m->d_grad + m->w_off[3 * L], m->d_grad + m->n_params,
                              m->d_grad + m->n_params + 1, 1, m->d_ws, m->d_occH[L - 1], m->d_occG[L - 1], st);
        int wl = -1, tt = 0;
        for (int l = L - 1; l >= 0 && !rc; --l) {
            const int cout = m->hidden[l], cin = l > 0 ? m->hidden[l - 1] : 1;
            const float* Hin = l > 0 ? m->d_H[l - 1] : m->d_X;
            if (l > 0 && wait_fill(m, L + (l - 1), s)) {
                rc = 1;
                break;
            }
            g_scone_hints.in_wl = wl;
            g_scone_hints.in_tt = tt;
            if (l == L - 1) g_scone_hints.in_bm = m->d_bmG;
            rc = scone_layer_backward(cx, m->act, b, cin, cout, m->d_G[l], Hin, m->d_w + m->w_off[3 * l],
                                      m->d_w + m->w_off[3 * l + 1], m->d_w + m->w_off[3 * l + 2], l > 0 ? m->d_G[l - 1] : nullptr,
                                      m->d_grad + m->w_off[3 * l], 1, m->d_ws, m->d_occG[l], l > 0 ? m->d_occH[l - 1] : nullptr,
                                      l > 0 ? m->d_occG[l - 1] : nullptr, m->d_occS, st);
            wl = g_scone_hints.out_wl;
            tt = g_scone_hints.out_tt;
        }
    }
    return finish_call(m, rc, user_st);
}

extern "C" int scone_model_forward_host(scone_model* m, int32_t B, const int32_t* ptr, const int32_t* edge, const float* val,
                                        const int32_t* last, float* logprobs_out, void* st) {
    SCONE_REQUIRE(m && ptr && last && logprobs_out && B >= 0, "scone_model_forward_host: bad arguments");
    if (B == 0) return 0;
    cudaStream_t s = as_stream(st);
    const int64_t nnz = ptr[B];
    int rc = ensure_staging(m, B, nnz);
    if (rc) return rc;
    SCONE_CUDA(cudaMemcpyAsync(m->d_ptr, ptr, (B + 1) * sizeof(int32_t), cudaMemcpyHostToDevice, s));
    SCONE_CUDA(cudaMemcpyAsync(m->d_last, last, B * sizeof(int32_t), cudaMemcpyHostToDevice, s));
    if (fused_host_overlap_ok(m, B, nnz)) {
        rc = fused_host_overlapped(m, B, ptr, edge, val, m->d_logp_all, false, 0, s);
    } else {
        SCONE_CUDA(cudaMemcpyAsync(m->d_edge, edge, nnz * sizeof(int32_t), cudaMemcpyHostToDevice, s));
        SCONE_CUDA(cudaMemcpyAsync(m->d_val, val, nnz * sizeof(float), cudaMemcpyHostToDevice, s));
        rc = scone_model_forward_dev(m, B, m->d_ptr, m->d_edge, m->d_val, m->d_last, m->d_logp_all, st);
    }
    if (rc) return rc;
    SCONE_CUDA(cudaMemcpyAsync(logprobs_out, m->d_logp_all, (size_t)B * m->cx->D * sizeof(float), cudaMemcpyDeviceToHost, s));
    int overflow = 0;
    if (m->d_overflow) SCONE_CUDA(cudaMemcpyAsync(&overflow, m->d_overflow, sizeof(int), cudaMemcpyDeviceToHost, s));
    SCONE_CUDA(cudaStreamSynchronize(s));
    if (overflow) {
        cudaMemset(m->d_overflow, 0, sizeof(int));
        m->cone_clean = false;
        scone_set_error("scone_model: a micro-batch exceeded a row-list capacity (%d rows per compact tensor, %d cone edges per trajectory "
                        "and layer); the log-probs are incomplete — use a smaller micro-batch or scone_model_set_pipeline(m, 2 / 0)",
                        m->row_cap, 2048);
        return 4;
    }
    return 0;
}

extern "C" int scone_accuracy_dev(int32_t B, int32_t D, const float* logprobs, const int32_t* n_nbrs, const int32_t* target_idx,
                                  const float* mask, int32_t* out, void* st) {
    SCONE_REQUIRE(B >= 0 && D >= 1 && out && (B == 0 || (logprobs && n_nbrs && target_idx && mask)), "scone_accuracy_dev: bad arguments");
    return scone_accuracy_launch(B, D, logprobs, n_nbrs, target_idx, mask, out, as_stream(st));
}

extern "C" int scone_model_accuracy_host(scone_model* m, int32_t B, const int32_t* ptr, const int32_t* edge, const float* val,
                                         const int32_t* last, const int32_t* n_nbrs, const int32_t* tgt, const float* mask,
                                         int32_t* out_host, void* st) {
    SCONE_REQUIRE(m && out_host && B >= 0 && (B == 0 || (ptr && last && n_nbrs && tgt && mask)), "scone_model_accuracy_host: bad arguments");
    out_host[0] = out_host[1] = 0;
    if (B == 0) return 0;
    cudaStream_t s = as_stream(st);
    const int64_t nnz = ptr[B];
    int rc = ensure_staging(m, B, nnz);
    if (rc) return rc;
    SCONE_CUDA(cudaMemcpyAsync(m->d_ptr, ptr, (B + 1) * sizeof(int32_t), cudaMemcpyHostToDevice, s));
    if (nnz) {
        SCONE_CUDA(cudaMemcpyAsync(m->d_edge, edge, nnz * sizeof(int32_t), cudaMemcpyHostToDevice, s));
        SCONE_CUDA(cudaMemcpyAsync(m->d_val, val, nnz * sizeof(float), cudaMemcpyHostToDevice, s));
    }
    SCONE_CUDA(cudaMemcpyAsync(m->d_last, last, B * sizeof(int32_t), cudaMemcpyHostToDevice, s));
    SCONE_CUDA(cudaMemcpyAsync(m->d_nn, n_nbrs, B * sizeof(int32_t), cudaMemcpyHostToDevice, s));
    SCONE_CUDA(cudaMemcpyAsync(m->d_tgt, tgt, B * sizeof(int32_t), cudaMemcpyHostToDevice, s));
    SCONE_CUDA(cudaMemcpyAsync(m->d_mask, mask, B * sizeof(float), cudaMemcpyHostToDevice, s));
    rc = scone_model_forward_dev(m, B, m->d_ptr, m->d_edge, m->d_val, m->d_last, m->d_logp_all, st);
    if (rc) return rc;
    rc = scone_accuracy_launch(B, m->cx->D, m->d_logp_all, m->d_nn, m->d_tgt, m->d_mask, m->d_acc, s);
    if (rc) return rc;
    SCONE_CUDA(cudaMemcpyAsync(out_host, m->d_acc, 2 * sizeof(int32_t), cudaMemcpyDeviceToHost, s));
    int overflow = 0;
    if (m->d_overflow) SCONE_CUDA(cudaMemcpyAsync(&overflow, m->d_overflow, sizeof(int), cudaMemcpyDeviceToHost, s));
    SCONE_CUDA(cudaStreamSynchronize(s));
    if (overflow) {
        cudaMemset(m->d_overflow, 0, sizeof(int));
        m->cone_clean = false;
        scone_set_error("scone_model: a micro-batch exceeded a row-list capacity; the accuracy is incomplete — use a smaller micro-batch or "
                        "scone_model_set_pipeline(m, 2 / 0)");
        return 4;
    }
    return 0;
}

extern "C" int scone_model_eval_host(scone_model* m, int32_t B, const int32_t* ptr, const int32_t* edge, const float* val,
                                     const int32_t* last, const int32_t* n_nbrs, const int32_t* tgt, const float* mask,
                                     int32_t* choice_out, int32_t* acc_out, float* nll_out, void* st) {
    SCONE_REQUIRE(m && B >= 0 && (B == 0 || (ptr && last)), "scone_model_eval_host: bad arguments");
    SCONE_REQUIRE(!choice_out || n_nbrs, "scone_model_eval_host: choice_out needs n_nbrs");
    SCONE_REQUIRE(!acc_out || (n_nbrs && tgt && mask), "scone_model_eval_host: acc_out needs n_nbrs, target_idx and mask");
    SCONE_REQUIRE(!nll_out || (tgt && mask), "scone_model_eval_host: nll_out needs target_idx and mask");
    if (acc_out) acc_out[0] = acc_out[1] = 0;
    if (nll_out) nll_out[0] = nll_out[1] = 0.f;
    m->eval_B = 0;
    if (B == 0) return 0;
    cudaStream_t s = as_stream(st);
    const int64_t nnz = ptr[B];
    int rc = ensure_staging(m, B, nnz);
    if (rc) return rc;
    if (!m->d_choice || m->cap_choice < B) {
        cudaFree(m->d_choice); cudaFree(m->d_rand);
        m->d_choice = m->d_rand = nullptr;
        SCONE_CUDA(cudaMalloc((void**)&m->d_choice, (size_t)m->cap_B * sizeof(int32_t)));
        SCONE_CUDA(cudaMalloc((void**)&m->d_rand, (size_t)m->cap_B * sizeof(int32_t)));
        m->cap_choice = m->cap_B;
    }
    if (!m->d_evalf) SCONE_CUDA(cudaMalloc((void**)&m->d_evalf, 4 * sizeof(float)));
    SCONE_CUDA(cudaMemcpyAsync(m->d_ptr, ptr, (B + 1) * sizeof(int32_t), cudaMemcpyHostToDevice, s));
    if (nnz) {
        SCONE_CUDA(cudaMemcpyAsync(m->d_edge, edge, nnz * sizeof(int32_t), cudaMemcpyHostToDevice, s));
        SCONE_CUDA(cudaMemcpyAsync(m->d_val, val, nnz * sizeof(float), cudaMemcpyHostToDevice, s));
    }
    SCONE_CUDA(cudaMemcpyAsync(m->d_last, last, B * sizeof(int32_t), cudaMemcpyHostToDevice, s));
    if (n_nbrs) SCONE_CUDA(cudaMemcpyAsync(m->d_nn, n_nbrs, B * sizeof(int32_t), cudaMemcpyHostToDevice, s));
    if (tgt) SCONE_CUDA(cudaMemcpyAsync(m->d_tgt, tgt, B * sizeof(int32_t), cudaMemcpyHostToDevice, s));
    if (mask) SCONE_CUDA(cudaMemcpyAsync(m->d_mask, mask, B * sizeof(float), cudaMemcpyHostToDevice, s));
    rc = scone_model_forward_dev(m, B, m->d_ptr, m->d_edge, m->d_val, m->d_last, m->d_logp_all, st);
    if (rc) return rc;
    const int D = m->cx->D;
    if (choice_out) {
        if (scone_predict_launch(B, D, m->d_logp_all, m->d_nn, m->d_choice, s)) return 1;
        SCONE_CUDA(cudaMemcpyAsync(choice_out, m->d_choice, B * sizeof(int32_t), cudaMemcpyDeviceToHost, s));
    }
    if (acc_out) {
        if (scone_accuracy_launch(B, D, m->d_logp_all, m->d_nn, m->d_tgt, m->d_mask, m->d_acc, s)) return 1;
        SCONE_CUDA(cudaMemcpyAsync(acc_out, m->d_acc, 2 * sizeof(int32_t), cudaMemcpyDeviceToHost, s));
    }
    if (nll_out) {
        if (scone_nll_launch(B, D, m->d_logp_all, m->d_tgt, m->d_mask, m->d_evalf, s)) return 1;
        SCONE_CUDA(cudaMemcpyAsync(nll_out, m->d_evalf, 2 * sizeof(float), cudaMemcpyDeviceToHost, s));
    }
    int overflow = 0;
    if (m->d_overflow) SCONE_CUDA(cudaMemcpyAsync(&overflow, m->d_overflow, sizeof(int), cudaMemcpyDeviceToHost, s));
    SCONE_CUDA(cudaStreamSynchronize(s));
    if (overflow) {
        cudaMemset(m->d_overflow, 0, sizeof(int));
        m->cone_clean = false;
        scone_set_error("scone_model: a micro-batch exceeded a row-list capacity; the evaluation is incomplete — use a smaller micro-batch or "
                        "another pipeline");
        return 4;
    }
    m->eval_B = B;
    return 0;
}

extern "C" int scone_model_two_target_host(scone_model* m, int32_t B, const int32_t* true_idx, const int32_t* rand_idx, int32_t* out, void* st) {
    SCONE_REQUIRE(m && out && B >= 0 && (B == 0 || (true_idx && rand_idx)), "scone_model_two_target_host: bad arguments");
    SCONE_REQUIRE(B == m->eval_B, "scone_model_two_target_host: call scone_model_eval_host (with n_nbrs and mask) on the same %d trajectories first", B);
    out[0] = out[1] = 0;
    if (B == 0) return 0;
    cudaStream_t s = as_stream(st);
    SCONE_CUDA(cudaMemcpyAsync(m->d_tgt, true_idx, B * sizeof(int32_t), cudaMemcpyHostToDevice, s));
    SCONE_CUDA(cudaMemcpyAsync(m->d_rand, rand_idx, B * sizeof(int32_t), cudaMemcpyHostToDevice, s));
    if (scone_two_target_launch(B, m->cx->D, m->d_logp_all, m->d_nn, m->d_tgt, m->d_rand, m->d_mask, m->d_acc, s)) return 1;
    SCONE_CUDA(cudaMemcpyAsync(out, m->d_acc, 2 * sizeof(int32_t), cudaMemcpyDeviceToHost, s));
    SCONE_CUDA(cudaStreamSynchronize(s));
    return 0;
}

extern "C" int scone_model_loss_grad_host(scone_model* m, int32_t B, const int32_t* ptr, const int32_t* edge, const float* val,
                                          const int32_t* last, const int32_t* tgt, const float* mask, int32_t zero_first,
                                          void* st) {
    SCONE_REQUIRE(m && ptr && last && tgt && mask && B >= 0, "scone_model_loss_grad_host: bad arguments");
    cudaStream_t s = as_stream(st);
    const int64_t nnz = B > 0 ? ptr[B] : 0;
    int rc = ensure_staging(m, B, nnz);
    if (rc) return rc;
    SCONE_CUDA(cudaMemcpyAsync(m->d_ptr, ptr, (B + 1) * sizeof(int32_t), cudaMemcpyHostToDevice, s));
    if (B) {
        SCONE_CUDA(cudaMemcpyAsync(m->d_last, last, B * sizeof(int32_t), cudaMemcpyHostToDevice, s));
        SCONE_CUDA(cudaMemcpyAsync(m->d_tgt, tgt, B * sizeof(int32_t), cudaMemcpyHostToDevice, s));
        SCONE_CUDA(cudaMemcpyAsync(m->d_mask, mask, B * sizeof(float), cudaMemcpyHostToDevice, s));
    }
    if (fused_host_overlap_ok(m, B, nnz)) return fused_host_overlapped(m, B, ptr, edge, val, nullptr, true, zero_first, s);
    if (nnz) {
        SCONE_CUDA(cudaMemcpyAsync(m->d_edge, edge, nnz * sizeof(int32_t), cudaMemcpyHostToDevice, s));
        SCONE_CUDA(cudaMemcpyAsync(m->d_val, val, nnz * sizeof(float), cudaMemcpyHostToDevice, s));
    }
    return scone_model_loss_grad_dev(m, B, m->d_ptr, m->d_edge, m->d_val, m->d_last, m->d_tgt, m->d_mask, zero_first, st);
}

extern "C" int scone_model_read_grads_async(scone_model* m, float* out_pinned, void* st) {
    SCONE_REQUIRE(m && out_pinned, "scone_model_read_grads_async: NULL argument");
    SCONE_CUDA(cudaMemcpyAsync(out_pinned, m->d_grad, (m->n_params + 2) * sizeof(float), cudaMemcpyDeviceToHost, as_stream(st)));
    return 0;
}

extern "C" int scone_model_read_grads(scone_model* m, float* out, void* st) {
    SCONE_REQUIRE(m && out, "scone_model_read_grads: NULL argument");
    cudaStream_t s = as_stream(st);
    SCONE_CUDA(cudaMemcpyAsync(out, m->d_grad, (m->n_params + 2) * sizeof(float), cudaMemcpyDeviceToHost, s));
    int overflow = 0;
    if (m->d_overflow) SCONE_CUDA(cudaMemcpyAsync(&overflow, m->d_overflow, sizeof(int), cudaMemcpyDeviceToHost, s));
    SCONE_CUDA(cudaStreamSynchronize(s));
    if (overflow) {
        cudaMemset(m->d_overflow, 0, sizeof(int));
        m->cone_clean = false;
        scone_set_error("scone_model: a micro-batch exceeded a row-list capacity (%d rows per compact tensor, %d rows of the backward's A "
                        "buffer, 2048 cone edges per trajectory and layer); the gradients are incomplete — use a smaller micro-batch or "
                        "scone_model_set_pipeline(m, 2 / 0)", m->row_cap, m->a_cap);
        return 4;
    }
    return 0;
}

extern "C" int scone_model_plan_dev(scone_model* m, int32_t B, const int32_t* ptr, const int32_t* edge, const float* val, const int32_t* last,
                                    void* user_st) {
    SCONE_REQUIRE(m && B >= 0 && (B == 0 || (ptr && last)), "scone_model_plan_dev: bad arguments");
    SCONE_REQUIRE(m->fused != nullptr, "scone_model_plan_dev: planned sets need the fused pipeline (uniform width 16 / 32, <= 3 layers)");
    if (fork_to_compute(m, user_st)) return 1;
    const int rc = scone_fused_plan_set(m->cx, m->fused, B, ptr, edge, val, last, m->d_overflow, m->compute);
    return finish_call(m, rc, user_st);
}

extern "C" int scone_model_plan_host(scone_model* m, int32_t B, const int32_t* ptr, const int32_t* edge, const float* val, const int32_t* last,
                                     void* st) {
    SCONE_REQUIRE(m && B >= 0 && (B == 0 || (ptr && last)), "scone_model_plan_host: bad arguments");
    SCONE_REQUIRE(m->fused != nullptr, "scone_model_plan_host: planned sets need the fused pipeline (uniform width 16 / 32, <= 3 layers)");
    cudaStream_t s = as_stream(st);
    const int64_t nnz = B > 0 ? ptr[B] : 0;
    int rc = ensure_staging(m, B, nnz);
    if (rc) return rc;
    SCONE_CUDA(cudaMemcpyAsync(m->d_ptr, ptr, (B + 1) * sizeof(int32_t), cudaMemcpyHostToDevice, s));
    if (nnz) {
        SCONE_CUDA(cudaMemcpyAsync(m->d_edge, edge, nnz * sizeof(int32_t), cudaMemcpyHostToDevice, s));
        SCONE_CUDA(cudaMemcpyAsync(m->d_val, val, nnz * sizeof(float), cudaMemcpyHostToDevice, s));
    }
    if (B) SCONE_CUDA(cudaMemcpyAsync(m->d_last, last, B * sizeof(int32_t), cudaMemcpyHostToDevice, s));
    rc = scone_model_plan_dev(m, B, m->d_ptr, m->d_edge, m->d_val, m->d_last, st);
    if (rc) return rc;
    return scone_model_check_overflow(m, st);
}

extern "C" int scone_model_loss_grad_planned_dev(scone_model* m, int32_t n, const int32_t* rows_dev, const int32_t* tgt_dev, const float* mask_dev,
                                                 int32_t zero_first, void* user_st) {
    SCONE_REQUIRE(m && n >= 0 && (n == 0 || (tgt_dev && mask_dev)), "scone_model_loss_grad_planned_dev: bad arguments");
    SCONE_REQUIRE(m->fused != nullptr, "scone_model_loss_grad_planned_dev: no fused pipeline");
    if (fork_to_compute(m, user_st)) return 1;
    cudaStream_t s = m->compute;
    if (zero_first) SCONE_CUDA(cudaMemsetAsync(m->d_grad, 0, (m->n_params + 2) * sizeof(float), s));
    const int rc = scone_fused_run_planned(m->cx, m->fused, m->act, n, rows_dev, m->d_w, m->w_off.data(), nullptr, tgt_dev, mask_dev, m->d_grad,
                                           g_scone_prof, s);
    return finish_call(m, rc, user_st);
}

extern "C" int scone_model_loss_grad_planned_host(scone_model* m, int32_t n, const int32_t* rows, const int32_t* tgt, const float* mask,
                                                  int32_t zero_first, void* st) {
    SCONE_REQUIRE(m && n >= 0 && (n == 0 || (tgt && mask)), "scone_model_loss_grad_planned_host: bad arguments");
    cudaStream_t s = as_stream(st);
    int rc = ensure_staging(m, n, 0);
    if (rc) return rc;
    if (n) {
        if (rows) SCONE_CUDA(cudaMemcpyAsync(m->d_nn, rows, n * sizeof(int32_t), cudaMemcpyHostToDevice, s));
        SCONE_CUDA(cudaMemcpyAsync(m->d_tgt, tgt, n * sizeof(int32_t), cudaMemcpyHostToDevice, s));
        SCONE_CUDA(cudaMemcpyAsync(m->d_mask, mask, n * sizeof(float), cudaMemcpyHostToDevice, s));
    }
    return scone_model_loss_grad_planned_dev(m, n, rows ? m->d_nn : nullptr, m->d_tgt, m->d_mask, zero_first, st);
}

extern "C" int scone_model_forward_planned_host(scone_model* m, int32_t n, const int32_t* rows, float* logprobs_out, void* st) {
    SCONE_REQUIRE(m && n >= 0 && (n == 0 || logprobs_out), "scone_model_forward_planned_host: bad arguments");
    SCONE_REQUIRE(m->fused != nullptr, "scone_model_forward_planned_host: no fused pipeline");
    if (n == 0) return 0;
    cudaStream_t s = as_stream(st);
    int rc = ensure_staging(m, n, 0);
    if (rc) return rc;
    if (rows) SCONE_CUDA(cudaMemcpyAsync(m->d_nn, rows, n * sizeof(int32_t), cudaMemcpyHostToDevice, s));
    if (fork_to_compute(m, st)) return 1;
    rc = scone_fused_run_planned(m->cx, m->fused, m->act, n, rows ? m->d_nn : nullptr, m->d_w, m->w_off.data(), m->d_logp_all, nullptr, nullptr,
                                 nullptr, false, m->compute);
    rc = finish_call(m, rc, st);
    if (rc) return rc;
    SCONE_CUDA(cudaMemcpyAsync(logprobs_out, m->d_logp_all, (size_t)n * m->cx->D * sizeof(float), cudaMemcpyDeviceToHost, s));
    SCONE_CUDA(cudaStreamSynchronize(s));
    return 0;
}

extern "C" int scone_model_check_overflow(scone_model* m, void* st) {
    SCONE_REQUIRE(m != nullptr, "scone_model_check_overflow: NULL model");
    int overflow = 0;
    cudaStream_t s = as_stream(st);
    if (m->d_overflow) SCONE_CUDA(cudaMemcpyAsync(&overflow, m->d_overflow, sizeof(int), cudaMemcpyDeviceToHost, s));
    SCONE_CUDA(cudaStreamSynchronize(s));
    if (overflow) {
        cudaMemset(m->d_overflow, 0, sizeof(int));
        m->cone_clean = false;
        scone_set_error("scone_model: a micro-batch exceeded a row-list capacity (%d rows per compact tensor, %d rows of the backward's A "
                        "buffer, 2048 cone edges per trajectory and layer); results since the last check are incomplete and Adam steps were "
                        "skipped — use a smaller micro-batch or another pipeline", m->row_cap, m->a_cap);
        return 4;
    }
    return 0;
}

extern "C" int scone_model_set_weights_keep_state(scone_model* m, const float* w, void* st) {
    SCONE_REQUIRE(m && w, "scone_model_set_weights_keep_state: NULL argument");
    SCONE_CUDA(cudaMemcpyAsync(m->d_w, w, m->n_params * sizeof(float), cudaMemcpyHostToDevice, as_stream(st)));
    return 0;
}

extern "C" int scone_model_fused_info(const scone_model* m, int32_t* out ) {
    SCONE_REQUIRE(m && out, "scone_model_fused_info: NULL argument");
    for (int i = 0; i < 16; ++i) out[i] = 0;
    if (!m->fused) return 0;
    const FusedState* f = m->fused;
    out[0] = 1; out[1] = f->bound_cone; out[2] = f->bound_list; out[3] = f->HS; out[4] = f->chunk; out[5] = f->cap_rows;
    out[6] = (int32_t)(f->plan_smem / 1024); out[7] = (int32_t)(f->traj_smem_small / 1024);
    out[8] = f->HS0; out[9] = f->LV0; out[10] = (int32_t)(f->plan_smem0 / 1024); out[11] = f->two_tiers ? 1 : 0;
    out[12] = f->tb_rows ? (int32_t)std::max<unsigned long long>(1, f->tb_bytes >> 20) : 0; out[13] = (int32_t)(f->arena_words >> 20);
    out[14] = (int32_t)std::min<unsigned long long>(f->cone_entries >> 10, 0x7fffffffull); out[15] = scone_fused_last_retries(m->fused);
    return 0;
}

extern "C" int scone_model_fused_read(scone_model* m, int32_t t, int32_t* hdr_out, uint32_t off, int32_t words, uint32_t* arena_out) {
    SCONE_REQUIRE(m && m->fused, "scone_model_fused_read: the model has no fused pipeline");
    SCONE_REQUIRE(t >= 0 && t < m->fused->chunk && (uint64_t)off + (uint64_t)(words > 0 ? words : 0) <= m->fused->arena_words,
                  "scone_model_fused_read: out of range");
    return scone_fused_read(m->fused, t, hdr_out, off, words, arena_out);
}

extern "C" int scone_model_read_rows_done(scone_model* m, int64_t* out ) {
    SCONE_REQUIRE(m && out, "scone_model_read_rows_done: NULL argument");
    out[0] = out[1] = 0;
    if (!m->fused) return 0;
    unsigned long long v[2];
    SCONE_CUDA(cudaMemcpy(v, m->fused->d_rows_done, sizeof(v), cudaMemcpyDeviceToHost));
    SCONE_CUDA(cudaMemset(m->fused->d_rows_done, 0, sizeof(v)));
    out[0] = (int64_t)v[0];
    out[1] = (int64_t)v[1];
    return 0;
}

extern "C" int scone_umma_status(void* st) { return scone_umma_check(as_stream(st)); }

extern "C" int scone_model_dp_adam_step(scone_model* m, scone_dp* dp, int32_t step, float lr, float wd, void* st) {
    SCONE_REQUIRE(m && dp && step >= 0, "scone_model_dp_adam_step: bad arguments");
    return scone_dp_allreduce_adam(dp, m->d_w, m->d_m, m->d_v, m->d_grad, m->n_params, m->d_overflow, step, lr, wd, as_stream(st));
}

extern "C" int scone_model_adam_step(scone_model* m, int32_t step, float lr, float wd, void* st) {
    SCONE_REQUIRE(m && step >= 0, "scone_model_adam_step: bad arguments");
    return scone_adam_launch(m->d_w, m->d_m, m->d_v, m->d_grad, m->n_params, step, lr, wd, st, m->d_overflow);
}
```

scone_gcn_b200/csrc/scone_plan_table.cu:

```cuda
#include <algorithm>
#include <cstdlib>
#include <vector>
#include "common.cuh"
#include "fused.cuh"

namespace {

constexpr int kTbThreads = 256;
constexpr int kTbHS = 32768;
constexpr int kTbLC = 16384;
constexpr uint32_t kEdgeMask = 0x3FFFFFFFu;
constexpr uint32_t kEmpty = 0xFFFFFFFFu;
constexpr uint32_t kNoRow = 0xFFFFu;
constexpr int kTbMaxD = 128;
constexpr int kTbBuckets = 1024;

__device__ __forceinline__ int align2(int x) { return (x + 1) & ~1; }

struct BuildArgs {
    const int32_t* nbrhoods;
    const int32_t* inc_ptr;
    const int2* inc_ent;
    const int32_t* mptr;
    const int2* ment;
    int N, D, L;
    int* stats;
    int* cnt_m;
    unsigned* cnt_e;
    int* cnt_p;
    const unsigned* cone_ptr;
    uint32_t* keys;
    int with_rows;
    const unsigned long long* node_off;
    unsigned* rowptr;
    int2* ent;
    const unsigned* pair_ptr;
    int2* pairs;
    int* pair_off;
};

__device__ __forceinline__ int find_sorted(const uint32_t* s, int m, uint32_t e) {
    int lo = 0, hi = m;
    while (lo < hi) {
        const int mid = (lo + hi) >> 1;
        if ((s[mid] & kEdgeMask) < e) lo = mid + 1;
        else hi = mid;
    }
    return lo < m && (s[lo] & kEdgeMask) == e ? lo : -1;
}

__global__ void __launch_bounds__(kTbThreads) table_build_kernel(const BuildArgs a) {
    extern __shared__ __align__(16) unsigned char sm[];
    uint32_t* hk = reinterpret_cast<uint32_t*>(sm);
    uint32_t* list = hk + kTbHS;
    __shared__ int s_ptr[kTbMaxD], s_off[kTbMaxD + 1];
    __shared__ int s_nlist, s_m, s_n1, s_ovf, s_nat[kFusedMaxL + 2], s_warp[kTbThreads / 32];
    __shared__ unsigned s_etot;
    const int tid = threadIdx.x, lane = tid & 31, ql = tid & 3;
    const unsigned qmask = 0xFu << (lane & ~3);
    const int node = blockIdx.x, D = a.D, L = a.L;
    const bool fill = a.keys != nullptr;
    for (int i = tid; i < kTbHS; i += kTbThreads) hk[i] = kEmpty;
    if (tid == 0) {
        s_nlist = s_m = s_n1 = s_ovf = 0;
        s_etot = 0u;
    }
    for (int j = tid; j < D; j += kTbThreads) {
        const int nbr = a.nbrhoods[(size_t)node * D + j];
        s_ptr[j] = nbr >= 0 ? a.inc_ptr[nbr] : -1;
        s_off[j + 1] = nbr >= 0 ? a.inc_ptr[nbr + 1] - a.inc_ptr[nbr] : 0;
    }
    __syncthreads();
    if (tid == 0) {
        s_off[0] = 0;
        for (int j = 0; j < D; ++j) s_off[j + 1] += s_off[j];
    }
    __syncthreads();
    const int total_pairs = s_off[D];
    auto slot_of = [&](int i) {
        int j = 0;
        while (j + 1 < D && s_off[j + 1] <= i) ++j;
        return j;
    };
    const unsigned c0 = fill ? a.cone_ptr[node] : 0u;
    const int cap = fill ? (int)(a.cone_ptr[node + 1] - c0) : kTbLC;
    uint32_t* kout = fill ? a.keys + c0 : nullptr;
    auto home = [](uint32_t e) { return (e * 2654435761u) >> 17; };
    auto level_of = [&](uint32_t e) -> int {
        unsigned h = home(e);
        for (;;) {
            const uint32_t k = hk[h];
            if (k == kEmpty) return -1;
            if ((k & kEdgeMask) == e) return (int)(k >> 30);
            h = (h + 1) & (kTbHS - 1);
        }
    };
    auto add = [&](uint32_t e, int lv) {
        unsigned h = home(e);
        const uint32_t val = e | ((uint32_t)lv << 30);
        for (int probes = 0; probes < kTbHS; ++probes) {
            const uint32_t old = atomicCAS(&hk[h], kEmpty, val);
            if (old == kEmpty) {
                const int k = atomicAdd(&s_m, 1);
                if (k >= cap) s_ovf = 1;
                else if (kout != nullptr) kout[k] = val;
                if (lv >= 1) {
                    atomicAdd(&s_n1, 1);
                    const int pos = atomicAdd(&s_nlist, 1);
                    if (pos < kTbLC) list[pos] = e;
                    else s_ovf = 1;
                }
                return;
            }
            if ((old & kEdgeMask) == e) return;
            h = (h + 1) & (kTbHS - 1);
        }
        s_ovf = 1;
    };
    for (int i = tid; i < total_pairs; i += kTbThreads) {
        const int j = slot_of(i);
        add((uint32_t)a.inc_ent[s_ptr[j] + (i - s_off[j])].x, L);
    }
    __syncthreads();
    if (tid == 0) s_nat[L] = min(s_nlist, kTbLC);
    __syncthreads();
    int f0 = 0;
    for (int lv = L - 1; lv >= 0; --lv) {
        const int f1 = s_nat[lv + 1];
        if (!s_ovf)
            for (int i = f0 + (tid >> 2); i < f1; i += kTbThreads / 4) {
                const int e = (int)list[i];
                const int p1 = a.mptr[e + 1];
                for (int q = a.mptr[e] + ql; q < p1; q += 4) add((uint32_t)a.ment[q].x, lv);
            }
        __syncthreads();
        if (tid == 0) s_nat[lv] = min(s_nlist, kTbLC);
        __syncthreads();
        f0 = f1;
    }
    const int m = s_m;
    const bool bad = s_ovf != 0 || m > cap;
    if (!fill) {
        if (!bad) {
            unsigned c = 0;
            const int n1 = s_nlist;
            for (int i = tid >> 2; i < n1; i += kTbThreads / 4) {
                const int e = (int)list[i];
                const int p1 = a.mptr[e + 1];
                for (int q = a.mptr[e] + ql; q < p1; q += 4) c += level_of((uint32_t)a.ment[q].x) == 0 ? 2u : 1u;
            }
            if (c) atomicAdd(&s_etot, c);
        }
        __syncthreads();
        if (tid == 0) {
            a.cnt_m[node] = bad ? 0 : m;
            a.cnt_e[node] = bad ? 0u : s_etot;
            a.cnt_p[node] = total_pairs;
            if (bad) a.stats[2] = 1;
            else {
                atomicMax(&a.stats[0], m);
                atomicMax(&a.stats[1], s_n1);
                atomicMax(&a.stats[3], total_pairs);
                atomicAdd(&a.stats[4 + min(kTbBuckets - 1, m / 32)], 1);
            }
        }
        return;
    }
    if (bad) {
        if (tid == 0) a.stats[2] = 1;
        return;
    }
    __syncthreads();
    uint32_t* tmp = hk;
    for (int i = tid; i < m; i += kTbThreads) tmp[i] = kout[i];
    __syncthreads();
    uint32_t* sorted = list;
    for (int k = tid; k < m; k += kTbThreads) {
        const uint32_t v = tmp[k], e = v & kEdgeMask;
        int r = 0;
        for (int q = 0; q < m; ++q) r += (tmp[q] & kEdgeMask) < e ? 1 : 0;
        sorted[r] = v;
    }
    __syncthreads();
    for (int i = tid; i < m; i += kTbThreads) kout[i] = sorted[i];
    if (a.with_rows) {
        for (int i = tid; i < total_pairs; i += kTbThreads) {
            const int j = slot_of(i);
            const int2 es = a.inc_ent[s_ptr[j] + (i - s_off[j])];
            const int li = find_sorted(sorted, m, (uint32_t)es.x);
            a.pairs[a.pair_ptr[node] + i] = make_int2((int)((li >= 0 ? (uint32_t)li : kNoRow) | ((uint32_t)j << 16)), es.y);
        }
        for (int j = tid; j <= D; j += kTbThreads) a.pair_off[(size_t)node * (D + 1) + j] = s_off[j];
    }
    if (!a.with_rows) return;
    int* cnt = reinterpret_cast<int*>(hk);
    for (int i = tid >> 2; i < m; i += kTbThreads / 4) {
        const uint32_t v = sorted[i];
        const int e = (int)(v & kEdgeMask);
        const bool full = (v >> 30) >= 1;
        const int p1 = a.mptr[e + 1];
        int c = 0;
        for (int q = a.mptr[e] + ql; q < p1; q += 4) {
            const int li = find_sorted(sorted, m, (uint32_t)a.ment[q].x);
            if (li >= 0 && (full || (sorted[li] >> 30) >= 1)) ++c;
        }
        c += __shfl_xor_sync(qmask, c, 1);
        c += __shfl_xor_sync(qmask, c, 2);
        if (ql == 0) cnt[i] = c;
    }
    __syncthreads();
    const int total = fused_block_scan_excl<kTbThreads>(cnt, m, s_warp);
    const unsigned long long nb = a.node_off[node];
    if ((unsigned long long)total != a.node_off[node + 1] - nb) {
        if (tid == 0) a.stats[2] = 2;
        return;
    }
    unsigned* rp = a.rowptr + c0 + node;
    for (int i = tid; i <= m; i += kTbThreads) rp[i] = (unsigned)cnt[i];
    int2* ent = a.ent + nb;
    for (int i = tid >> 2; i < m; i += kTbThreads / 4) {
        const uint32_t v = sorted[i];
        const int e = (int)(v & kEdgeMask);
        const bool full = (v >> 30) >= 1;
        const int p0 = a.mptr[e], p1 = a.mptr[e + 1];
        int base = cnt[i];
        for (int q0 = p0; q0 < p1; q0 += 4) {
            const int q = q0 + ql;
            int li = -1;
            int2 en = make_int2(0, 0);
            if (q < p1) {
                en = a.ment[q];
                li = find_sorted(sorted, m, (uint32_t)en.x);
                if (li >= 0 && !(full || (sorted[li] >> 30) >= 1)) li = -1;
            }
            const bool valid = li >= 0;
            const unsigned bits = (__ballot_sync(qmask, valid) >> (lane & ~3)) & 0xFu;
            if (valid) ent[base + __popc(bits & ((1u << ql) - 1u))] = make_int2((int)((uint32_t)li | (li == i ? 0x80000000u : 0u)), en.y);
            base += __popc(bits);
        }
    }
}

__host__ __device__ inline size_t table_plan_smem(int M, int LV) {
    const size_t W = (size_t)M / 32;
    return (size_t)M * 8 + (3 * W + W + 2) * 4 + (4 * (size_t)LV + 8) * 4 + 3 * (size_t)M * 2 + 3 * (size_t)LV * 2 + (size_t)M + 16;
}

template <int THREADS>
__device__ __forceinline__ void table_plan_trajectory(const PlanArgs& a, const int t, unsigned char* sm) {
    constexpr int QUADS = THREADS / 4;
    const int M = a.M, LV = a.LV, L = a.L, D = a.D, W = M >> 5;
    uint32_t* keys = reinterpret_cast<uint32_t*>(sm);
    float* x = reinterpret_cast<float*>(keys + M);
    unsigned* bits = reinterpret_cast<unsigned*>(x + M);
    int* wpre = reinterpret_cast<int*>(bits + 3 * W);
    int* cnt = wpre + W + 2;
    uint16_t* idx = reinterpret_cast<uint16_t*>(cnt + 4 * LV + 8);
    uint16_t* byr = idx + 3 * M;
    uint8_t* lv = reinterpret_cast<uint8_t*>(byr + 3 * LV);
    __shared__ int s_n, s_ovf, s_warp[THREADS / 32];
    __shared__ unsigned s_piece;

    const int tid = threadIdx.x, lane = tid & 31, warp = tid >> 5, ql = tid & 3;
    const unsigned qmask = 0xFu << (lane & ~3);
    int* hdr = a.hdr + (size_t)t * kFusedHdrW;
    auto give_up = [&]() {
        if (tid == 0) {
            if (a.retry != nullptr) {
                hdr[0] = kFusedFlagRetry;
                a.retry[atomicAdd(a.n_retry, 1)] = t;
            } else {
                hdr[0] = kFusedFlagOverflow;
                *a.overflow = 1;
            }
        }
    };
    const int last = a.last_nodes[t];
    const bool last_ok = last >= 0 && last < a.N;
    const unsigned c0 = last_ok ? a.cone_ptr[last] : 0u;
    const int m = last_ok ? (int)(a.cone_ptr[last + 1] - c0) : 0;
    if (m > M) {
        give_up();
        return;
    }
    const int Wm = (m + 31) >> 5;
    for (int i = tid; i < m; i += THREADS) {
        const uint32_t k = a.cone_ent[c0 + i];
        keys[i] = k & kEdgeMask;
        lv[i] = (uint8_t)(k >> 30);
        x[i] = 0.f;
        idx[i] = idx[M + i] = idx[2 * M + i] = (uint16_t)kNoRow;
    }
    for (int w = tid; w < Wm; w += THREADS) bits[w] = bits[W + w] = bits[2 * W + w] = 0u;
    if (tid == 0) s_ovf = 0;
    const unsigned* rp = a.tb_rowptr + c0 + (last_ok ? last : 0);
    const int2* ent = a.tb_ent + (last_ok ? a.node_off[last] : 0ull);
    const int fp0 = a.traj_ptr[t], fp1 = a.traj_ptr[t + 1];
    __syncthreads();
    auto rank_live = [&](int l) -> int {
        __syncthreads();
        const unsigned* bl = bits + (l - 1) * W;
        uint16_t* il = idx + (l - 1) * M;
        uint16_t* byrank = byr + (l - 1) * LV;
        if (warp == 0) {
            int run = 0;
            for (int base = 0; base < Wm; base += 32) {
                const int w = base + lane < Wm ? __popc(bl[base + lane]) : 0;
                int inc = w;
#pragma unroll
                for (int o = 1; o < 32; o <<= 1) {
                    const int v = __shfl_up_sync(0xffffffffu, inc, o);
                    if (lane >= o) inc += v;
                }
                if (base + lane < Wm) wpre[base + lane] = run + inc - w;
                run += __shfl_sync(0xffffffffu, inc, 31);
            }
            if (lane == 0) {
                s_n = run;
                if (run > LV) s_ovf = 1;
            }
        }
        __syncthreads();
        const int n = s_n;
        if (n <= LV)
            for (int j = tid; j < m; j += THREADS) {
                const unsigned wd = bl[j >> 5];
                if ((wd >> (j & 31)) & 1u) {
                    const int r = wpre[j >> 5] + __popc(wd & ((1u << (j & 31)) - 1u));
                    il[j] = (uint16_t)r;
                    byrank[r] = (uint16_t)j;
                }
            }
        return n;
    };

    for (int p = fp0 + tid; p < fp1; p += THREADS) {
        const int eo = a.flow_edge[p];
        if (eo < 0 || eo >= a.E) continue;
        const uint32_t e = (uint32_t)a.rank[eo];
        int lo = 0, hi = m;
        while (lo < hi) {
            const int mid = (lo + hi) >> 1;
            if (keys[mid] < e) lo = mid + 1;
            else hi = mid;
        }
        if (lo >= m || keys[lo] != e) continue;
        const float v = a.flow_val[p];
        x[lo] = v;
        if (v == 0.f) continue;
        const unsigned q1 = rp[lo + 1];
        for (unsigned q = rp[lo]; q < q1; ++q) {
            const int j = ent[q].x & 0xFFFF;
            if (lv[j] >= 1) atomicOr(&bits[j >> 5], 1u << (j & 31));
        }
    }
    int n_l[kFusedMaxL + 2] = {0, 0, 0, 0, 0};
    int pbF[kFusedMaxL + 2] = {0, 0, 0, 0, 0}, pbT[kFusedMaxL + 2] = {0, 0, 0, 0, 0}, rbase[kFusedMaxL + 2] = {0, 0, 0, 0, 0};
    int n_prog_rows = 0, n_rows = 0, ptr_words = 0;
    n_l[1] = rank_live(1);
    for (int s = 1; s <= L && !s_ovf; ++s) {
        __syncthreads();
        const int ns = n_l[s];
        rbase[s] = n_rows;
        n_rows += ns;
        if (s >= 2) {
            pbF[s] = n_prog_rows;
            n_prog_rows += ns;
            ptr_words += align2(ns + 1);
        }
        if (s < L) {
            pbT[s] = n_prog_rows;
            n_prog_rows += ns;
            ptr_words += align2(ns + 1);
        }
        if (s == 1 && L == 1) break;
        const uint16_t* brow = byr + (s - 1) * LV;
        const uint16_t* idx_prev = idx + (s >= 2 ? s - 2 : 0) * M;
        unsigned* bn = bits + (s < L ? s : 0) * W;
        int* cF = cnt + pbF[s];
        int* cT = cnt + pbT[s];
        const int lnext = s + 1;
        for (int r = tid >> 2; r < ns; r += QUADS) {
            const int i = brow[r];
            const unsigned q1 = rp[i + 1];
            int f = 0, tr = 0;
            for (unsigned q = rp[i] + ql; q < q1; q += 4) {
                const int j = ent[q].x & 0xFFFF;
                if (s >= 2 && idx_prev[j] != (uint16_t)kNoRow) ++f;
                if (s < L && lv[j] >= lnext) {
                    ++tr;
                    atomicOr(&bn[j >> 5], 1u << (j & 31));
                }
            }
            f += __shfl_xor_sync(qmask, f, 1);
            f += __shfl_xor_sync(qmask, f, 2);
            tr += __shfl_xor_sync(qmask, tr, 1);
            tr += __shfl_xor_sync(qmask, tr, 2);
            if (ql == 0) {
                if (s >= 2) cF[r] = f;
                if (s < L) cT[r] = tr;
            }
        }
        if (s < L) n_l[s + 1] = rank_live(s + 1);
    }
    __syncthreads();
    if (s_ovf) {
        give_up();
        return;
    }
    for (int s = L + 1; s <= kFusedMaxL + 1; ++s) rbase[s] = n_rows;
    auto layer_of = [&](int row) { return row < rbase[2] ? 1 : (row < rbase[3] ? 2 : 3); };
    const unsigned pp0 = last_ok ? a.pair_ptr[last] : 0u;
    const int total_pairs = last_ok ? (int)(a.pair_ptr[last + 1] - pp0) : 0;
    const int fixed_words = align2(3 * n_l[1]) + align2(D + 1) + 2 * total_pairs + ptr_words;
    int total_ent;
    {
        const int n = n_prog_rows;
        const int per = (n + THREADS - 1) / THREADS;
        const int lo = min(n, tid * per), hi = min(n, lo + per);
        int sum = 0;
        for (int i = lo; i < hi; ++i) sum += cnt[i];
        int inc = sum;
#pragma unroll
        for (int o = 1; o < 32; o <<= 1) {
            const int v = __shfl_up_sync(0xffffffffu, inc, o);
            if (lane >= o) inc += v;
        }
        if (lane == 31) s_warp[warp] = inc;
        __syncthreads();
        int base = 0, total = 0;
#pragma unroll
        for (int w = 0; w < THREADS / 32; ++w) {
            const int v = s_warp[w];
            if (w < warp) base += v;
            total += v;
        }
        int run = base + inc - sum;
        for (int i = lo; i < hi; ++i) {
            const int v = cnt[i];
            cnt[i] = run;
            run += v;
        }
        if (tid == 0) {
            cnt[n] = total;
            const unsigned long long w = (unsigned long long)(fixed_words + 2 * total);
            const unsigned long long o = atomicAdd(a.bump, w);
            if (o + w > a.arena_words) {
                s_ovf = 2;
                s_piece = 0u;
            } else {
                s_piece = (unsigned)o;
            }
        }
        __syncthreads();
        total_ent = total;
    }
    if (s_ovf) {
        if (tid == 0) {
            hdr[0] = kFusedFlagOverflow;
            *a.overflow = 1;
        }
        return;
    }
    const unsigned off_l1 = s_piece;
    const unsigned off_ro = off_l1 + (unsigned)align2(3 * n_l[1]);
    unsigned off_f[kFusedMaxL + 2] = {0, 0, 0, 0, 0}, off_b[kFusedMaxL + 2] = {0, 0, 0, 0, 0};
    int tot_f[kFusedMaxL + 2] = {0, 0, 0, 0, 0}, tot_b[kFusedMaxL + 2] = {0, 0, 0, 0, 0};
    {
        unsigned o = off_ro + (unsigned)(align2(D + 1) + 2 * total_pairs);
        for (int s = 1; s <= L; ++s) {
            if (s >= 2) {
                off_f[s] = o;
                tot_f[s] = cnt[pbF[s] + n_l[s]] - cnt[pbF[s]];
                o += (unsigned)(align2(n_l[s] + 1) + 2 * tot_f[s]);
            }
            if (s < L) {
                off_b[s + 1] = o;
                tot_b[s + 1] = cnt[pbT[s] + n_l[s]] - cnt[pbT[s]];
                o += (unsigned)(align2(n_l[s] + 1) + 2 * tot_b[s + 1]);
            }
        }
    }
    (void)total_ent;
    for (int s = 1; s <= L; ++s) {
        const int ns = n_l[s];
        if (s >= 2) {
            int* pF = reinterpret_cast<int*>(a.arena + off_f[s]);
            const int b0 = cnt[pbF[s]];
            for (int r = tid; r <= ns; r += THREADS) pF[r] = cnt[pbF[s] + r] - b0;
        }
        if (s < L) {
            int* pT = reinterpret_cast<int*>(a.arena + off_b[s + 1]);
            const int b0 = cnt[pbT[s]];
            for (int r = tid; r <= ns; r += THREADS) pT[r] = cnt[pbT[s] + r] - b0;
        }
    }
    {
        float* l1dst = reinterpret_cast<float*>(a.arena + off_l1);
        for (int row = tid >> 2; row < n_rows; row += QUADS) {
            const int s = layer_of(row), r = row - rbase[s];
            const int i = byr[(s - 1) * LV + r];
            const uint16_t* idx_prev = idx + (s >= 2 ? s - 2 : 0) * M;
            const uint16_t* idx_next = idx + (s < L ? s : 0) * M;
            int2* eF = reinterpret_cast<int2*>(a.arena + off_f[s] + align2(n_l[s] + 1));
            int2* eT = reinterpret_cast<int2*>(a.arena + off_b[s < L ? s + 1 : 0] + align2(n_l[s] + 1));
            int baseF = s >= 2 ? cnt[pbF[s] + r] - cnt[pbF[s]] : 0, baseT = s < L ? cnt[pbT[s] + r] - cnt[pbT[s]] : 0;
            const unsigned q0r = rp[i], q1 = rp[i + 1];
            float a1 = 0.f, a2 = 0.f;
            for (unsigned q0 = q0r; q0 < q1; q0 += 4) {
                const unsigned q = q0 + ql;
                uint32_t rf = kNoRow, rt = kNoRow;
                int2 en = make_int2(0, 0);
                if (q < q1) {
                    en = ent[q];
                    const int j = en.x & 0xFFFF;
                    if (s >= 2) rf = idx_prev[j];
                    if (s < L) rt = idx_next[j];
                    if (s == 1) {
                        const float xj = x[j];
                        if (xj != 0.f) {
                            a1 = fmaf((float)(short)(en.y & 0xffff), xj, a1);
                            a2 = fmaf((float)(en.y >> 16), xj, a2);
                        }
                    }
                }
                const uint32_t own = (uint32_t)en.x & 0x80000000u;
                if (s >= 2) {
                    const unsigned b = (__ballot_sync(qmask, rf != kNoRow) >> (lane & ~3)) & 0xFu;
                    if (rf != kNoRow) eF[baseF + __popc(b & ((1u << ql) - 1u))] = make_int2((int)(rf | own), en.y);
                    baseF += __popc(b);
                }
                if (s < L) {
                    const unsigned b = (__ballot_sync(qmask, rt != kNoRow) >> (lane & ~3)) & 0xFu;
                    if (rt != kNoRow) eT[baseT + __popc(b & ((1u << ql) - 1u))] = make_int2((int)(rt | own), en.y);
                    baseT += __popc(b);
                }
            }
            if (s == 1) {
#pragma unroll
                for (int o = 1; o < 4; o <<= 1) {
                    a1 += __shfl_xor_sync(qmask, a1, o);
                    a2 += __shfl_xor_sync(qmask, a2, o);
                }
                if (ql == 0) {
                    l1dst[3 * r + 0] = x[i];
                    l1dst[3 * r + 1] = a1;
                    l1dst[3 * r + 2] = a2;
                }
            }
        }
    }
    {
        const uint16_t* idxL = idx + (L - 1) * M;
        int* pdst = reinterpret_cast<int*>(a.arena + off_ro);
        int2* edst = reinterpret_cast<int2*>(a.arena + off_ro + align2(D + 1));
        for (int j = tid; j <= D; j += THREADS) pdst[j] = last_ok ? a.pair_off[(size_t)last * (D + 1) + j] : 0;
        for (int i = tid; i < total_pairs; i += THREADS) {
            const int2 pr = a.tb_pairs[pp0 + i];
            const uint32_t li = (uint32_t)pr.x & 0xFFFFu;
            const uint32_t r = li != kNoRow ? (uint32_t)idxL[li] : kNoRow;
            edst[i] = make_int2((int)(r | ((uint32_t)pr.x & 0xFFFF0000u)), pr.y);
        }
    }
    if (tid == 0) {
        hdr[0] = 0;
        for (int l = 1; l <= kFusedMaxL; ++l) hdr[l] = l <= L ? n_l[l] : 0;
        hdr[4] = (int)off_l1;
        for (int l = 2; l <= kFusedMaxL; ++l) {
            hdr[5 + (l - 2)] = (int)off_f[l];
            hdr[7 + (l - 2)] = (int)off_b[l];
        }
        hdr[9] = (int)off_ro;
        hdr[10] = total_pairs;
        hdr[11] = m;
        hdr[12] = tot_f[2];
        hdr[13] = fp1 - fp0;
        hdr[14] = tot_f[3];
        hdr[15] = min(tot_b[2], 0xFFFF) | (min(tot_b[3], 0xFFFF) << 16);
    }
}

template <int THREADS>
__global__ void __launch_bounds__(THREADS) table_plan_kernel(const PlanArgs a) {
    extern __shared__ __align__(16) unsigned char sm[];
    const int n_work = a.tier == 0 ? a.n_work : *a.n_in;
    for (int w = blockIdx.x; w < n_work; w += gridDim.x) {
        table_plan_trajectory<THREADS>(a, a.tier == 0 ? a.t0 + w : a.in_list[w], sm);
        __syncthreads();
    }
}

constexpr int kTier1Threads = 512;
constexpr size_t kMaxTablePlanSmem = 220 * 1024;

}

void scone_table_destroy(FusedState* f) {
    cudaFree(f->d_cone_ptr); cudaFree(f->d_cone_ent); cudaFree(f->d_node_off); cudaFree(f->d_tb_rowptr); cudaFree(f->d_tb_ent);
    cudaFree(f->d_pair_ptr); cudaFree(f->d_tb_pairs); cudaFree(f->d_pair_off);
    f->d_cone_ptr = nullptr; f->d_cone_ent = nullptr; f->d_node_off = nullptr; f->d_tb_rowptr = nullptr; f->d_tb_ent = nullptr;
    f->d_pair_ptr = nullptr; f->d_tb_pairs = nullptr; f->d_pair_off = nullptr;
    f->tb_rows = false;
}

int scone_table_build(const scone_complex* cx, FusedState* f, int L, bool* ok) {
    *ok = false;
    const int N = cx->N, D = cx->D;
    if (D > kTbMaxD || N < 1) return 0;
    const int n_stats = 4 + kTbBuckets;
    SCONE_CUDA(cudaMalloc((void**)&f->d_stats, n_stats * sizeof(int)));
    SCONE_CUDA(cudaMemset(f->d_stats, 0, n_stats * sizeof(int)));
    const size_t smem = (size_t)kTbHS * 4 + (size_t)kTbLC * 4;
    SCONE_CUDA(cudaFuncSetAttribute(table_build_kernel, cudaFuncAttributeMaxDynamicSharedMemorySize, (int)smem));
    int* d_cnt_m = nullptr;
    unsigned* d_cnt_e = nullptr;
    int* d_cnt_p = nullptr;
    SCONE_CUDA(cudaMalloc((void**)&d_cnt_m, (size_t)N * sizeof(int)));
    SCONE_CUDA(cudaMalloc((void**)&d_cnt_e, (size_t)N * sizeof(unsigned)));
    SCONE_CUDA(cudaMalloc((void**)&d_cnt_p, (size_t)N * sizeof(int)));
    BuildArgs a{};
    a.nbrhoods = cx->d_nbrhoods; a.inc_ptr = cx->d_inc_ptr; a.inc_ent = cx->d_inc_ent; a.mptr = cx->d_mptr; a.ment = cx->d_ment;
    a.N = N; a.D = D; a.L = L; a.stats = f->d_stats;
    a.cnt_m = d_cnt_m; a.cnt_e = d_cnt_e; a.cnt_p = d_cnt_p;
    table_build_kernel<<<N, kTbThreads, smem>>>(a);
    SCONE_LAUNCHED();
    std::vector<int> st(n_stats), cm((size_t)N), cp((size_t)N);
    std::vector<unsigned> ce((size_t)N);
    SCONE_CUDA(cudaMemcpy(st.data(), f->d_stats, n_stats * sizeof(int), cudaMemcpyDeviceToHost));
    SCONE_CUDA(cudaMemcpy(cm.data(), d_cnt_m, (size_t)N * sizeof(int), cudaMemcpyDeviceToHost));
    SCONE_CUDA(cudaMemcpy(ce.data(), d_cnt_e, (size_t)N * sizeof(unsigned), cudaMemcpyDeviceToHost));
    SCONE_CUDA(cudaMemcpy(cp.data(), d_cnt_p, (size_t)N * sizeof(int), cudaMemcpyDeviceToHost));
    cudaFree(d_cnt_m); cudaFree(d_cnt_e); cudaFree(d_cnt_p);
    std::vector<unsigned> cone_ptr((size_t)N + 1), pair_ptr((size_t)N + 1);
    std::vector<unsigned long long> node_off((size_t)N + 1);
    unsigned long long tm = 0, te = 0, tp = 0;
    for (int n = 0; n < N; ++n) {
        cone_ptr[n] = (unsigned)tm; node_off[n] = te; pair_ptr[n] = (unsigned)tp;
        tm += (unsigned long long)cm[n]; te += ce[n]; tp += (unsigned long long)cp[n];
    }
    if (st[2] || tm + (unsigned long long)N + 1 >= (1ull << 32) || tp >= (1ull << 32)) return 0;
    cone_ptr[N] = (unsigned)tm; node_off[N] = te; pair_ptr[N] = (unsigned)tp;
    f->cone_entries = tm;
    int quantile999 = 0;
    f->bound_cone = st[0] > 0 ? st[0] : 1;
    f->bound_list = st[1] > 0 ? st[1] : 1;
    {
        long long acc = 0, want = ((long long)N * 99 + 99) / 100;
        int q0 = 32 * kTbBuckets;
        for (int b = 0; b < kTbBuckets; ++b) {
            acc += st[4 + b];
            if (acc >= want) {
                q0 = 32 * (b + 1);
                break;
            }
        }
        f->quantile_cone = std::min(q0, f->bound_cone);
        acc = 0;
        want = ((long long)N * 999 + 999) / 1000;
        quantile999 = f->bound_cone;
        for (int b = 0; b < kTbBuckets; ++b) {
            acc += st[4 + b];
            if (acc >= want) {
                quantile999 = std::min(32 * (b + 1), f->bound_cone);
                break;
            }
        }
    }
    const unsigned long long bytes = te * 8 + (tm + (unsigned long long)N + 1) * 4 + tp * 8 + (unsigned long long)N * (D + 1) * 4 + ((unsigned long long)N + 1) * 16;
    bool want_rows = true;
    {
        const char* v = getenv("SCONE_FUSED_TABLE");
        if (v && *v == '0') want_rows = false;
        size_t free_b = 0, total_b = 0;
        SCONE_CUDA(cudaMemGetInfo(&free_b, &total_b));
        if (bytes > free_b / 3) want_rows = false;
        f->tbM = (f->bound_cone + 63) & ~63;
        f->tbLV = (f->bound_list + 63) & ~63;
        f->tb_smem = table_plan_smem(f->tbM, f->tbLV);
        if (f->tb_smem > kMaxTablePlanSmem || f->bound_cone >= 0xFFFF || f->bound_list >= 0xFFFF) want_rows = false;
    }
    SCONE_CUDA(cudaMalloc((void**)&f->d_cone_ptr, cone_ptr.size() * sizeof(unsigned)));
    SCONE_CUDA(cudaMalloc((void**)&f->d_cone_ent, (size_t)(tm ? tm : 1) * sizeof(uint32_t)));
    SCONE_CUDA(cudaMemcpy(f->d_cone_ptr, cone_ptr.data(), cone_ptr.size() * sizeof(unsigned), cudaMemcpyHostToDevice));
    a.cnt_m = nullptr; a.cnt_e = nullptr; a.cnt_p = nullptr;
    a.cone_ptr = f->d_cone_ptr; a.keys = f->d_cone_ent; a.with_rows = want_rows ? 1 : 0;
    if (want_rows) {
        SCONE_CUDA(cudaMalloc((void**)&f->d_node_off, node_off.size() * sizeof(unsigned long long)));
        SCONE_CUDA(cudaMalloc((void**)&f->d_tb_rowptr, (size_t)(tm + N + 1) * sizeof(unsigned)));
        SCONE_CUDA(cudaMalloc((void**)&f->d_tb_ent, (size_t)(te ? te : 1) * sizeof(int2)));
        SCONE_CUDA(cudaMalloc((void**)&f->d_pair_ptr, pair_ptr.size() * sizeof(unsigned)));
        SCONE_CUDA(cudaMalloc((void**)&f->d_tb_pairs, (size_t)(tp ? tp : 1) * sizeof(int2)));
        SCONE_CUDA(cudaMalloc((void**)&f->d_pair_off, (size_t)N * (D + 1) * sizeof(int)));
        SCONE_CUDA(cudaMemcpy(f->d_node_off, node_off.data(), node_off.size() * sizeof(unsigned long long), cudaMemcpyHostToDevice));
        SCONE_CUDA(cudaMemcpy(f->d_pair_ptr, pair_ptr.data(), pair_ptr.size() * sizeof(unsigned), cudaMemcpyHostToDevice));
        a.node_off = f->d_node_off; a.rowptr = f->d_tb_rowptr; a.ent = f->d_tb_ent;
        a.pair_ptr = f->d_pair_ptr; a.pairs = f->d_tb_pairs; a.pair_off = f->d_pair_off;
    }
    table_build_kernel<<<N, kTbThreads, smem>>>(a);
    SCONE_LAUNCHED();
    SCONE_CUDA(cudaDeviceSynchronize());
    SCONE_CUDA(cudaMemcpy(st.data(), f->d_stats, 4 * sizeof(int), cudaMemcpyDeviceToHost));
    if (st[2] == 1) return 0;
    if (st[2] == 2) {
        want_rows = false;
        SCONE_CUDA(cudaMemset(f->d_stats + 2, 0, sizeof(int)));
        cudaFree(f->d_node_off); cudaFree(f->d_tb_rowptr); cudaFree(f->d_tb_ent); cudaFree(f->d_pair_ptr); cudaFree(f->d_tb_pairs); cudaFree(f->d_pair_off);
        f->d_node_off = nullptr; f->d_tb_rowptr = nullptr; f->d_tb_ent = nullptr; f->d_pair_ptr = nullptr; f->d_tb_pairs = nullptr; f->d_pair_off = nullptr;
    }
    f->tb_rows = want_rows;
    if (want_rows) {
        f->tb_entries = te;
        f->tb_bytes = bytes;
        auto env_int = [](const char* name, int dflt) {
            const char* v = getenv(name);
            return v && *v ? atoi(v) : dflt;
        };
        f->tbM0 = std::min(f->tbM, (env_int("SCONE_TABLE_M0", f->quantile_cone) + 63) & ~63);
        f->tbLV0 = std::min(f->tbLV, (env_int("SCONE_TABLE_LV0", 192) + 63) & ~63);
        f->tb_two_tiers = f->tbM0 < f->tbM || f->tbLV0 < f->tbLV;
        f->tb_smem0 = table_plan_smem(f->tbM0, f->tbLV0);
        f->tbM1 = std::min(f->tbM, (env_int("SCONE_TABLE_M1", std::max(quantile999, 2 * f->tbM0)) + 63) & ~63);
        f->tbLV1 = std::min(f->tbLV, (env_int("SCONE_TABLE_LV1", 512) + 63) & ~63);
        f->tb_smem1 = table_plan_smem(f->tbM1, f->tbLV1);
        f->tb_mid_tier = f->tb_two_tiers && (f->tbM1 > f->tbM0 || f->tbLV1 > f->tbLV0) && 2 * f->tb_smem1 <= f->tb_smem;
        SCONE_CUDA(cudaFuncSetAttribute(table_plan_kernel<64>, cudaFuncAttributeMaxDynamicSharedMemorySize, (int)kMaxTablePlanSmem));
        SCONE_CUDA(cudaFuncSetAttribute(table_plan_kernel<128>, cudaFuncAttributeMaxDynamicSharedMemorySize, (int)kMaxTablePlanSmem));
        SCONE_CUDA(cudaFuncSetAttribute(table_plan_kernel<256>, cudaFuncAttributeMaxDynamicSharedMemorySize, (int)kMaxTablePlanSmem));
        SCONE_CUDA(cudaFuncSetAttribute(table_plan_kernel<kTier1Threads>, cudaFuncAttributeMaxDynamicSharedMemorySize, (int)kMaxTablePlanSmem));
    }
    *ok = true;
    return 0;
}

int scone_table_plan_launch(const FusedState* f, PlanArgs p, int b, int num_sms, cudaStream_t st, int phase) {
    const int f_chunk = f->chunk;
    p.cone_ptr = f->d_cone_ptr; p.cone_ent = f->d_cone_ent; p.node_off = f->d_node_off; p.tb_rowptr = f->d_tb_rowptr; p.tb_ent = f->d_tb_ent;
    p.pair_ptr = f->d_pair_ptr; p.tb_pairs = f->d_tb_pairs; p.pair_off = f->d_pair_off;
    p.tier = 0; p.n_work = b;
    p.M = f->tbM0; p.LV = f->tbLV0;
    int* list0 = p.retry;
    int* list1 = p.retry + f_chunk;
    int* cnt0 = p.n_retry;
    int* cnt1 = p.n_retry + 1;
    p.retry = f->tb_two_tiers ? list0 : nullptr;
    p.n_retry = cnt0;
    if (phase != 1) {
        static const int t0 = [] { const char* v = getenv("SCONE_TABLE_T0"); return v && *v ? atoi(v) : 128; }();
        if (t0 == 64) table_plan_kernel<64><<<b, 64, f->tb_smem0, st>>>(p);
        else if (t0 == 256) table_plan_kernel<256><<<b, 256, f->tb_smem0, st>>>(p);
        else table_plan_kernel<128><<<b, 128, f->tb_smem0, st>>>(p);
        SCONE_LAUNCHED();
    }
    if (!f->tb_two_tiers || phase == 0) return 0;
    const int* n_in = cnt0;
    const int* in_list = list0;
    if (f->tb_mid_tier) {
        p.tier = 1; p.M = f->tbM1; p.LV = f->tbLV1; p.n_in = n_in; p.in_list = in_list; p.retry = list1; p.n_retry = cnt1;
        const int per_sm = std::max(1, std::min(8, (int)((size_t)220 * 1024 / (f->tb_smem1 + 1024))));
        table_plan_kernel<256><<<std::min(b, per_sm * num_sms), 256, f->tb_smem1, st>>>(p);
        SCONE_LAUNCHED();
        n_in = cnt1;
        in_list = list1;
    }
    p.tier = 2; p.M = f->tbM; p.LV = f->tbLV; p.n_in = n_in; p.in_list = in_list; p.retry = nullptr; p.n_retry = cnt0;
    const int per_sm = std::max(1, std::min(4, (int)((size_t)220 * 1024 / (f->tb_smem + 1024))));
    table_plan_kernel<512><<<std::min(b, per_sm * num_sms), 512, f->tb_smem, st>>>(p);
    SCONE_LAUNCHED();
    return 0;
}
```

scone_gcn_b200/model.py:

```python
import ctypes as C

import numpy as np

from . import _lib


class SconeModel:
    def __init__(self, cx, hidden, micro_batch=64, zero_fill=False):
        self.cx = cx
        self.hidden = [int(h) for h in hidden]
        self.micro_batch = int(micro_batch)
        L = _lib.lib()
        harr = np.asarray(self.hidden, dtype=np.int32)
        h = C.c_void_p()
        _lib.check(L.scone_model_create(cx.handle, len(self.hidden), _lib.ptr(harr), self.micro_batch, C.byref(h)),
                   'scone_model_create')
        self.handle = h
        if zero_fill:
            self.set_zero_fill(True)
        self.n_params = L.scone_model_num_params(h)
        self.planned = 0
        self.shapes = []
        cin = 1
        for c in self.hidden:
            self.shapes += [(cin, c)] * 3
            cin = c
        self.shapes.append((cin, 1))

    def set_zero_fill(self, on):
        _lib.check(_lib.lib().scone_model_set_zero_fill(self.handle, int(bool(on))), 'scone_model_set_zero_fill')

    @property
    def pipeline(self):
        return int(_lib.lib().scone_model_get_pipeline(self.handle))

    def set_pipeline(self, which):
        _lib.check(_lib.lib().scone_model_set_pipeline(self.handle, int(which)), 'scone_model_set_pipeline')

    def fused_info(self):
        out = np.zeros(16, np.int32)
        _lib.check(_lib.lib().scone_model_fused_info(self.handle, _lib.ptr(out)), 'scone_model_fused_info')
        if not out[0]:
            return None
        keys = ['available', 'bound_cone', 'bound_list', 'hash_slots', 'chunk', 'cap_rows', 'plan_smem_kb', 'traj_smem_kb', 'hash_slots_tier0',
                'live_rows_tier0', 'plan_smem_tier0_kb', 'two_tiers', 'table_plan_mb', 'arena_mwords', 'cone_table_kentries', 'retries_last_chunk']
        return dict(zip(keys, (int(v) for v in out)))

    def fused_header(self, t):
        hdr = np.zeros(16, np.int32)
        _lib.check(_lib.lib().scone_model_fused_read(self.handle, int(t), _lib.ptr(hdr), 0, 0, None), 'scone_model_fused_read')
        return hdr

    def check_overflow(self, stream=None):
        _lib.check(_lib.lib().scone_model_check_overflow(self.handle, stream), 'scone_model_check_overflow')

    def flatten(self, weights):
        assert len(weights) == len(self.shapes), 'wrong number of weights'
        parts = []
        for w, s in zip(weights, self.shapes):
            w = np.asarray(w, dtype=np.float32)
            assert w.shape == s, 'weight shape %s, expected %s' % (w.shape, s)
            parts.append(w.ravel())
        return np.ascontiguousarray(np.concatenate(parts))

    def unflatten(self, flat):
        out, off = [], 0
        for s in self.shapes:
            n = s[0] * s[1]
            out.append(flat[off:off + n].reshape(s).copy())
            off += n
        return out

    def set_weights(self, weights, reset_adam=True, stream=None):
        flat = self.flatten(weights)
        if reset_adam:
            _lib.check(_lib.lib().scone_model_set_weights(self.handle, _lib.ptr(flat)), 'scone_model_set_weights')
        else:
            self._pending_weights = flat
            _lib.check(_lib.lib().scone_model_set_weights_keep_state(self.handle, _lib.ptr(flat), stream),
                       'scone_model_set_weights_keep_state')

    def get_weights(self):
        flat = np.zeros(self.n_params, np.float32)
        _lib.check(_lib.lib().scone_model_get_weights(self.handle, _lib.ptr(flat)), 'scone_model_get_weights')
        return self.unflatten(flat)

    def forward(self, traj_ptr, flow_edge, flow_val, last_nodes, stream=None):
        B = len(last_nodes)
        out = np.zeros((B, self.cx.D), np.float32)
        traj_ptr = np.ascontiguousarray(traj_ptr, np.int32)
        flow_edge = np.ascontiguousarray(flow_edge, np.int32)
        flow_val = np.ascontiguousarray(flow_val, np.float32)
        last_nodes = np.ascontiguousarray(last_nodes, np.int32)
        _lib.check(_lib.lib().scone_model_forward_host(self.handle, B, _lib.ptr(traj_ptr), _lib.ptr(flow_edge),
                                                       _lib.ptr(flow_val), _lib.ptr(last_nodes), _lib.ptr(out), stream),
                   'scone_model_forward_host')
        return out

    def loss_grad(self, traj_ptr, flow_edge, flow_val, last_nodes, target_idx, mask, zero_first=True, stream=None,
                  read=True):
        B = len(last_nodes)
        a = [np.ascontiguousarray(traj_ptr, np.int32), np.ascontiguousarray(flow_edge, np.int32),
             np.ascontiguousarray(flow_val, np.float32), np.ascontiguousarray(last_nodes, np.int32),
             np.ascontiguousarray(target_idx, np.int32), np.ascontiguousarray(mask, np.float32)]
        _lib.check(_lib.lib().scone_model_loss_grad_host(self.handle, B, *[_lib.ptr(x) for x in a], int(zero_first), stream),
                   'scone_model_loss_grad_host')
        return self.read_grads(stream) if read else None

    def accuracy(self, traj_ptr, flow_edge, flow_val, last_nodes, n_nbrs, target_idx, mask, stream=None):
        B = len(last_nodes)
        a = [np.ascontiguousarray(traj_ptr, np.int32), np.ascontiguousarray(flow_edge, np.int32),
             np.ascontiguousarray(flow_val, np.float32), np.ascontiguousarray(last_nodes, np.int32),
             np.ascontiguousarray(n_nbrs, np.int32), np.ascontiguousarray(target_idx, np.int32),
             np.ascontiguousarray(mask, np.float32)]
        out = np.zeros(2, np.int32)
        _lib.check(_lib.lib().scone_model_accuracy_host(self.handle, B, *[_lib.ptr(x) for x in a], _lib.ptr(out), stream),
                   'scone_model_accuracy_host')
        return int(out[0]), int(out[1])

    def plan(self, traj_ptr, flow_edge, flow_val, last_nodes, stream=None):
        if self.pipeline != 4:
            return False
        B = len(last_nodes)
        a = [np.ascontiguousarray(traj_ptr, np.int32), np.ascontiguousarray(flow_edge, np.int32),
             np.ascontiguousarray(flow_val, np.float32), np.ascontiguousarray(last_nodes, np.int32)]
        _lib.check(_lib.lib().scone_model_plan_host(self.handle, B, *[_lib.ptr(x) for x in a], stream), 'scone_model_plan_host')
        self.planned = B
        return True

    def loss_grad_planned(self, rows, target_idx, mask, zero_first=True, stream=None, read=True):
        n = len(target_idx)
        r = None if rows is None else np.ascontiguousarray(rows, np.int32)
        t, k = np.ascontiguousarray(target_idx, np.int32), np.ascontiguousarray(mask, np.float32)
        _lib.check(_lib.lib().scone_model_loss_grad_planned_host(self.handle, n, _lib.ptr(r), _lib.ptr(t), _lib.ptr(k), int(zero_first), stream),
                   'scone_model_loss_grad_planned_host')
        return self.read_grads(stream) if read else None

    def forward_planned(self, rows=None, n=None, stream=None):
        r = None if rows is None else np.ascontiguousarray(rows, np.int32)
        n = len(r) if r is not None else (self.planned if n is None else n)
        out = np.zeros((n, self.cx.D), np.float32)
        _lib.check(_lib.lib().scone_model_forward_planned_host(self.handle, n, _lib.ptr(r), _lib.ptr(out), stream),
                   'scone_model_forward_planned_host')
        return out

    def evaluate(self, traj_ptr, flow_edge, flow_val, last_nodes, n_nbrs=None, target_idx=None, mask=None, want_choice=False,
                 want_accuracy=False, want_nll=False, stream=None):
        B = len(last_nodes)
        i32 = lambda a: None if a is None else np.ascontiguousarray(a, np.int32)
        a = [i32(traj_ptr), i32(flow_edge), np.ascontiguousarray(flow_val, np.float32), i32(last_nodes), i32(n_nbrs), i32(target_idx),
             None if mask is None else np.ascontiguousarray(mask, np.float32)]
        choice = np.zeros(B, np.int32) if want_choice else None
        acc = np.zeros(2, np.int32) if want_accuracy else None
        nll = np.zeros(2, np.float32) if want_nll else None
        _lib.check(_lib.lib().scone_model_eval_host(self.handle, B, *[_lib.ptr(x) for x in a], _lib.ptr(choice), _lib.ptr(acc), _lib.ptr(nll),
                                                    stream), 'scone_model_eval_host')
        out = {}
        if want_choice:
            out['choice'] = choice
        if want_accuracy:
            out['accuracy'] = (int(acc[0]), int(acc[1]))
        if want_nll:
            out['nll'] = (float(nll[0]), float(nll[1]))
        return out

    def two_target_counts(self, true_idx, rand_idx, stream=None):
        B = len(true_idx)
        t, r = np.ascontiguousarray(true_idx, np.int32), np.ascontiguousarray(rand_idx, np.int32)
        out = np.zeros(2, np.int32)
        _lib.check(_lib.lib().scone_model_two_target_host(self.handle, B, _lib.ptr(t), _lib.ptr(r), _lib.ptr(out), stream),
                   'scone_model_two_target_host')
        return int(out[0]), int(out[1])

    def read_grads(self, stream=None):
        buf = np.zeros(self.n_params + 2, np.float32)
        _lib.check(_lib.lib().scone_model_read_grads(self.handle, _lib.ptr(buf), stream), 'scone_model_read_grads')
        return buf

    def read_grads_async(self, pinned, stream=None):
        ptr = pinned.data_ptr() if hasattr(pinned, 'data_ptr') else pinned.ctypes.data
        _lib.check(_lib.lib().scone_model_read_grads_async(self.handle, ptr, stream), 'scone_model_read_grads_async')

    def adam_step(self, step, lr, weight_decay, stream=None):
        _lib.check(_lib.lib().scone_model_adam_step(self.handle, int(step), float(lr), float(weight_decay), stream),
                   'scone_model_adam_step')

    def grads_tensor(self):
        return _wrap_device_f32(_lib.lib().scone_model_grads_dev(self.handle), self.n_params + 2)

    def weights_tensor(self):
        return _wrap_device_f32(_lib.lib().scone_model_weights_dev(self.handle), self.n_params)

    def __del__(self):
        try:
            if getattr(self, 'handle', None):
                _lib.lib().scone_model_destroy(self.handle)
                self.handle = None
        except Exception:
            pass


class _CudaArray:

    def __init__(self, ptr, n):
        self.__cuda_array_interface__ = {'shape': (int(n),), 'typestr': '<f4', 'data': (int(ptr), False), 'version': 2}


def _wrap_device_f32(ptr, n):
    import torch
    return torch.as_tensor(_CudaArray(ptr, n), device='cuda')
```

Measured before the change: 7.445 million.

## Pre-classify trajectories into plan tiers per node and run tiers concurrently

Replaces the retry cascade, in which a trajectory first attempts the small tier-0 plan, gives up, and is retried at larger tiers. Each last node now gets a precomputed tier from cone and list sizes, and the tier-0 limits come from data quantiles instead of fixed constants. A classify kernel builds per-tier lists on a side stream while tier-0 blocks run on their own stream and skip trajectories owned by higher tiers. The streams are then joined before compute, which removes the wasted tier-0 attempts and overlaps the tiers, at the cost of extra streams, events and an oversized-case overflow path.

```diff
diff --git a/include/scone_b200.h b/include/scone_b200.h
--- a/include/scone_b200.h
+++ b/include/scone_b200.h
@@ -121,6 +121,7 @@
 int scone_model_check_overflow(scone_model* m, void* stream);
 int scone_model_set_weights_keep_state(scone_model* m, const float* weights_host, void* stream);
 int scone_model_fused_info(const scone_model* m, int32_t* out );
+int scone_model_fused_node_tiers(const scone_model* m, uint8_t* out , int32_t* sizes );
 int scone_model_fused_read(scone_model* m, int32_t t, int32_t* hdr_out , uint32_t off, int32_t words, uint32_t* arena_out);
 int scone_model_read_rows_done(scone_model* m, int64_t* out );
 
diff --git a/scone_gcn_b200/_lib.py b/scone_gcn_b200/_lib.py
--- a/scone_gcn_b200/_lib.py
+++ b/scone_gcn_b200/_lib.py
@@ -97,6 +97,7 @@
     'scone_model_forward_planned_host': (C.c_int, [_vp, _i32, _vp, _vp, _vp]),
     'scone_model_set_weights_keep_state': (C.c_int, [_vp, _vp, _vp]),
     'scone_model_fused_info': (C.c_int, [_vp, _vp]),
+    'scone_model_fused_node_tiers': (C.c_int, [_vp, _vp, _vp]),
     'scone_model_fused_read': (C.c_int, [_vp, _i32, _vp, C.c_uint32, _i32, _vp]),
     'scone_model_read_rows_done': (C.c_int, [_vp, _vp]),
 }
diff --git a/scone_gcn_b200/csrc/fused.cuh b/scone_gcn_b200/csrc/fused.cuh
--- a/scone_gcn_b200/csrc/fused.cuh
+++ b/scone_gcn_b200/csrc/fused.cuh
@@ -40,6 +40,7 @@
     int t0;
     const int* n_in;
     const int* in_list;
+    const uint8_t* node_tier;
     int* n_retry;
     int* retry;
 };
@@ -98,6 +99,13 @@
     int tbM0 = 0, tbLV0 = 0, tbM1 = 0, tbLV1 = 0, tbM = 0, tbLV = 0;
     size_t tb_smem0 = 0, tb_smem1 = 0, tb_smem = 0;
     bool tb_two_tiers = false, tb_mid_tier = false;
+    uint8_t* d_node_tier = nullptr;
+    int* d_tier_list = nullptr;
+    int* d_tier_cnt = nullptr;
+    cudaStream_t plan_side = nullptr;
+    cudaStream_t plan_tier0 = nullptr;
+    cudaEvent_t ev_plan_fork = nullptr, ev_plan_join = nullptr, ev_plan_join0 = nullptr;
+    bool plan_forked = false;
     int quantile_cone = 0;
     int HS = 0, LV = 0, EC = 0, hshift = 0;
     int HS0 = 0, LV0 = 0, EC0 = 0, hshift0 = 0;
@@ -129,7 +137,8 @@
 };
 
 int scone_table_build(const scone_complex* cx, FusedState* f, int L, bool* ok);
-int scone_table_plan_launch(const FusedState* f, PlanArgs p, int b, int num_sms, cudaStream_t st, int phase = 2);
+int scone_table_plan_launch(FusedState* f, PlanArgs p, int off, int b, int num_sms, cudaStream_t st);
+int scone_table_plan_join(FusedState* f, cudaStream_t st);
 void scone_table_destroy(FusedState* f);
 
 bool scone_fused_supported(const scone_complex* cx, int n_layers, const int32_t* hidden);
@@ -140,10 +149,8 @@
                     const int32_t* target_idx, const float* mask, float* grad, int* overflow, bool count_rows, cudaStream_t st);
 int scone_fused_begin(FusedState* f, cudaStream_t st);
 int scone_fused_plan_part(const scone_complex* cx, FusedState* f, int off, int b, const int32_t* traj_ptr, const int32_t* flow_edge,
-                          const float* flow_val, const int32_t* last_nodes, int* overflow, cudaStream_t st,
-                          bool defer_tiers = false);
-int scone_fused_plan_finish(const scone_complex* cx, FusedState* f, int B, const int32_t* traj_ptr, const int32_t* flow_edge,
-                            const float* flow_val, const int32_t* last_nodes, int* overflow, cudaStream_t st);
+                          const float* flow_val, const int32_t* last_nodes, int* overflow, cudaStream_t st);
+int scone_fused_plan_finish(FusedState* f, cudaStream_t st);
 int scone_fused_compute(const scone_complex* cx, FusedState* f, int act, int b, const float* W, const int64_t* w_off, float* logprobs,
                         const int32_t* target_idx, const float* mask, float* grad, bool count_rows, cudaStream_t st);
 int scone_fused_plan_set(const scone_complex* cx, FusedState* f, int B, const int32_t* traj_ptr, const int32_t* flow_edge,
@@ -152,3 +159,4 @@
                             float* logprobs, const int32_t* target_idx, const float* mask, float* grad, bool count_rows, cudaStream_t st);
 int scone_fused_last_retries(FusedState* f);
 int scone_fused_read(FusedState* f, int t, int* hdr_out, unsigned off, int words, uint32_t* arena_out);
+int scone_fused_node_tiers(const FusedState* f, int N, uint8_t* out);
diff --git a/scone_gcn_b200/csrc/scone_fused.cu b/scone_gcn_b200/csrc/scone_fused.cu
--- a/scone_gcn_b200/csrc/scone_fused.cu
+++ b/scone_gcn_b200/csrc/scone_fused.cu
@@ -1151,16 +1151,22 @@
     }
     SCONE_CUDA(cudaMalloc((void**)&f->d_arena, f->arena_words * sizeof(uint32_t)));
     SCONE_CUDA(cudaMalloc((void**)&f->d_hdr, (size_t)f->chunk * kFusedHdrW * sizeof(int)));
-    SCONE_CUDA(cudaMalloc((void**)&f->d_retry, 2 * (size_t)f->chunk * sizeof(int)));
     SCONE_CUDA(cudaMalloc((void**)&f->d_bump, 2 * sizeof(unsigned long long)));
+    if (f->tb_rows) {
+        if (f->d_node_tier) {
+            SCONE_CUDA(cudaMalloc((void**)&f->d_tier_list, 2 * (size_t)f->chunk * sizeof(int)));
+            SCONE_CUDA(cudaMalloc((void**)&f->d_tier_cnt, 2 * (size_t)f->chunk * sizeof(int)));
+        }
+    } else {
+        SCONE_CUDA(cudaMalloc((void**)&f->d_retry, (size_t)f->chunk * sizeof(int)));
+    }
     SCONE_CUDA(cudaMalloc((void**)&f->d_rows_done, 4 * sizeof(unsigned long long)));
     SCONE_CUDA(cudaMemset(f->d_rows_done, 0, 4 * sizeof(unsigned long long)));
     *out = f;
     return 0;
 }
 
-static int launch_plans(const scone_complex* cx, const FusedState* f, PlanArgs p, int b, cudaStream_t st) {
-    if (f->tb_rows) return scone_table_plan_launch(f, p, b, cx->num_sms, st);
+static int launch_hash_plans(const scone_complex* cx, const FusedState* f, PlanArgs p, int b, cudaStream_t st) {
     p.tier = 0; p.n_work = b;
     p.HS = f->HS0; p.LV = f->LV0; p.EC = f->EC0; p.hshift = f->hshift0;
     int* retry = p.retry;
@@ -1193,29 +1199,23 @@
 }
 
 int scone_fused_plan_part(const scone_complex* cx, FusedState* f, int off, int b, const int32_t* traj_ptr, const int32_t* flow_edge,
-                          const float* flow_val, const int32_t* last_nodes, int* overflow, cudaStream_t st, bool defer_tiers) {
+                          const float* flow_val, const int32_t* last_nodes, int* overflow, cudaStream_t st) {
     if (b <= 0) return 0;
     SCONE_REQUIRE(off >= 0 && off + b <= f->chunk, "scone_fused_plan_part: trajectories %d .. %d exceed the planned chunk of %d", off, off + b, f->chunk);
-    ScopedProf prof(SCONE_K_CONE, st);
-    if (defer_tiers && f->tb_rows) {
-        PlanArgs p = plan_args(cx, f, 0, traj_ptr, flow_edge, flow_val, last_nodes, overflow);
-        p.t0 = off;
-        return scone_table_plan_launch(f, p, b, cx->num_sms, st, 0);
-    }
+    if (f->tb_rows)
+        return scone_table_plan_launch(f, plan_args(cx, f, 0, traj_ptr, flow_edge, flow_val, last_nodes, overflow), off, b, cx->num_sms, st);
     if (off > 0) SCONE_CUDA(cudaMemsetAsync(f->d_bump + 1, 0, sizeof(unsigned long long), st));
-    return launch_plans(cx, f, plan_args(cx, f, off, traj_ptr, flow_edge, flow_val, last_nodes, overflow), b, st);
-}
-
-int scone_fused_plan_finish(const scone_complex* cx, FusedState* f, int B, const int32_t* traj_ptr, const int32_t* flow_edge,
-                            const float* flow_val, const int32_t* last_nodes, int* overflow, cudaStream_t st) {
-    if (B <= 0 || !f->tb_rows) return 0;
-    ScopedProf prof(SCONE_K_CONE, st);
-    return scone_table_plan_launch(f, plan_args(cx, f, 0, traj_ptr, flow_edge, flow_val, last_nodes, overflow), B, cx->num_sms, st, 1);
+    return launch_hash_plans(cx, f, plan_args(cx, f, off, traj_ptr, flow_edge, flow_val, last_nodes, overflow), b, st);
+}
+
+int scone_fused_plan_finish(FusedState* f, cudaStream_t st) {
+    return scone_table_plan_join(f, st);
 }
 
 int scone_fused_compute(const scone_complex* cx, FusedState* f, int act, int b, const float* W, const int64_t* w_off, float* logprobs,
                         const int32_t* target_idx, const float* mask, float* grad, bool count_rows, cudaStream_t st) {
     if (b <= 0) return 0;
+    if (scone_table_plan_join(f, st)) return 1;
     TrajArgs t;
     t.hdr = f->d_hdr; t.arena = f->d_arena; t.rows = nullptr; t.W = W;
     for (int i = 0; i <= 3 * kFusedMaxL; ++i) t.w_off[i] = i <= 3 * f->L ? (int)w_off[i] : 0;
@@ -1233,7 +1233,11 @@
     if (b <= 0) return 0;
     SCONE_REQUIRE(b <= f->chunk, "scone_fused_run: chunk of %d trajectories exceeds the planned %d", b, f->chunk);
     int rc = scone_fused_begin(f, st);
-    if (!rc) rc = scone_fused_plan_part(cx, f, 0, b, traj_ptr, flow_edge, flow_val, last_nodes, overflow, st);
+    {
+        ScopedProf prof(SCONE_K_CONE, st);
+        if (!rc) rc = scone_fused_plan_part(cx, f, 0, b, traj_ptr, flow_edge, flow_val, last_nodes, overflow, st);
+        if (!rc) rc = scone_fused_plan_finish(f, st);
+    }
     if (!rc) rc = scone_fused_compute(cx, f, act, b, W, w_off, logprobs, target_idx, mask, grad, count_rows, st);
     return rc;
 }
@@ -1265,11 +1269,18 @@
     ScopedProf prof(SCONE_K_CONE, st);
     for (int off = 0; off < B; off += f->chunk) {
         const int b = std::min(f->chunk, B - off);
-        SCONE_CUDA(cudaMemsetAsync(f->d_set_bump + 1, 0, sizeof(unsigned long long), st));
         p.traj_ptr = traj_ptr + off; p.last_nodes = last_nodes + off; p.hdr = f->d_set_hdr + (size_t)off * kFusedHdrW;
-        const int rc = launch_plans(cx, f, p, b, st);
+        int rc;
+        if (f->tb_rows) {
+            rc = scone_table_plan_launch(f, p, 0, b, cx->num_sms, st);
+        } else {
+            SCONE_CUDA(cudaMemsetAsync(f->d_set_bump + 1, 0, sizeof(unsigned long long), st));
+            rc = launch_hash_plans(cx, f, p, b, st);
+        }
         if (rc) return rc;
     }
+    const int rc = scone_table_plan_join(f, st);
+    if (rc) return rc;
     f->set_n = B;
     return 0;
 }
diff --git a/scone_gcn_b200/csrc/scone_model.cu b/scone_gcn_b200/csrc/scone_model.cu
--- a/scone_gcn_b200/csrc/scone_model.cu
+++ b/scone_gcn_b200/csrc/scone_model.cu
@@ -683,12 +683,14 @@
     cudaStream_t c = m->compute;
     if (grad && zero_first) SCONE_CUDA(cudaMemsetAsync(m->d_grad, 0, (m->n_params + 2) * sizeof(float), c));
     int rc = scone_fused_begin(m->fused, c);
-    for (int k = 0; k < kParts && !rc; ++k) {
-        SCONE_CUDA(cudaStreamWaitEvent(c, m->ev_part[k], 0));
-        rc = scone_fused_plan_part(m->cx, m->fused, b0[k], b0[k + 1] - b0[k], m->d_ptr, m->d_edge, m->d_val, m->d_last, m->d_overflow, c,
-                                   kParts > 1);
-    }
-    if (!rc && kParts > 1) rc = scone_fused_plan_finish(m->cx, m->fused, B, m->d_ptr, m->d_edge, m->d_val, m->d_last, m->d_overflow, c);
+    {
+        ScopedProf prof(SCONE_K_CONE, c);
+        for (int k = 0; k < kParts && !rc; ++k) {
+            SCONE_CUDA(cudaStreamWaitEvent(c, m->ev_part[k], 0));
+            rc = scone_fused_plan_part(m->cx, m->fused, b0[k], b0[k + 1] - b0[k], m->d_ptr, m->d_edge, m->d_val, m->d_last, m->d_overflow, c);
+        }
+        if (!rc) rc = scone_fused_plan_finish(m->fused, c);
+    }
     if (!rc) {
         SCONE_CUDA(cudaEventRecord(m->ev_plan_done, c));
         m->plan_done_epoch = m->staging_epoch;
@@ -1105,6 +1107,14 @@
     return 0;
 }
 
+extern "C" int scone_model_fused_node_tiers(const scone_model* m, uint8_t* out, int32_t* sizes) {
+    SCONE_REQUIRE(m && m->fused && out && sizes, "scone_model_fused_node_tiers: the model has no fused pipeline");
+    const FusedState* f = m->fused;
+    const int32_t v[6] = {f->tbM0, f->tbLV0, f->tb_mid_tier ? f->tbM1 : 0, f->tb_mid_tier ? f->tbLV1 : 0, f->tbM, f->tbLV};
+    for (int i = 0; i < 6; ++i) sizes[i] = f->tb_rows ? v[i] : 0;
+    return scone_fused_node_tiers(f, m->cx->N, out);
+}
+
 extern "C" int scone_model_fused_read(scone_model* m, int32_t t, int32_t* hdr_out, uint32_t off, int32_t words, uint32_t* arena_out) {
     SCONE_REQUIRE(m && m->fused, "scone_model_fused_read: the model has no fused pipeline");
     SCONE_REQUIRE(t >= 0 && t < m->fused->chunk && (uint64_t)off + (uint64_t)(words > 0 ? words : 0) <= m->fused->arena_words,
diff --git a/scone_gcn_b200/csrc/scone_plan_table.cu b/scone_gcn_b200/csrc/scone_plan_table.cu
--- a/scone_gcn_b200/csrc/scone_plan_table.cu
+++ b/scone_gcn_b200/csrc/scone_plan_table.cu
@@ -1,5 +1,6 @@
 #include <algorithm>
 #include <cstdlib>
+#include <cstring>
 #include <vector>
 #include "common.cuh"
 #include "fused.cuh"
@@ -28,6 +29,7 @@
     int* cnt_m;
     unsigned* cnt_e;
     int* cnt_p;
+    int* cnt_n1;
     const unsigned* cone_ptr;
     uint32_t* keys;
     int with_rows;
@@ -156,6 +158,7 @@
             a.cnt_m[node] = bad ? 0 : m;
             a.cnt_e[node] = bad ? 0u : s_etot;
             a.cnt_p[node] = total_pairs;
+            a.cnt_n1[node] = bad ? 0 : s_n1;
             if (bad) a.stats[2] = 1;
             else {
                 atomicMax(&a.stats[0], m);
@@ -266,13 +269,8 @@
     int* hdr = a.hdr + (size_t)t * kFusedHdrW;
     auto give_up = [&]() {
         if (tid == 0) {
-            if (a.retry != nullptr) {
-                hdr[0] = kFusedFlagRetry;
-                a.retry[atomicAdd(a.n_retry, 1)] = t;
-            } else {
-                hdr[0] = kFusedFlagOverflow;
-                *a.overflow = 1;
-            }
+            hdr[0] = kFusedFlagOverflow;
+            *a.overflow = 1;
         }
     };
     const int last = a.last_nodes[t];
@@ -583,10 +581,63 @@
 template <int THREADS>
 __global__ void __launch_bounds__(THREADS) table_plan_kernel(const PlanArgs a) {
     extern __shared__ __align__(16) unsigned char sm[];
-    const int n_work = a.tier == 0 ? a.n_work : *a.n_in;
+    if (a.tier == 0) {
+        const int t = a.t0 + blockIdx.x;
+        if (a.node_tier != nullptr) {
+            const int last = a.last_nodes[t];
+            if (last >= 0 && last < a.N && a.node_tier[last] != 0) return;
+        }
+        table_plan_trajectory<THREADS>(a, t, sm);
+        return;
+    }
+    const int n_work = *a.n_in;
     for (int w = blockIdx.x; w < n_work; w += gridDim.x) {
-        table_plan_trajectory<THREADS>(a, a.tier == 0 ? a.t0 + w : a.in_list[w], sm);
-        __syncthreads();
+        table_plan_trajectory<THREADS>(a, a.in_list[w], sm);
+        __syncthreads();
+    }
+}
+
+constexpr int kClassifyThreads = 1024;
+__global__ void __launch_bounds__(kClassifyThreads) table_classify_kernel(const int32_t* __restrict__ last_nodes, const uint8_t* __restrict__ node_tier,
+                                                                          int N, int t0, int b, int* __restrict__ list1, int* __restrict__ list2,
+                                                                          int* __restrict__ cnt1, int* __restrict__ cnt2) {
+    __shared__ int s_w[2][kClassifyThreads / 32];
+    __shared__ int s_base[2];
+    const int tid = threadIdx.x, lane = tid & 31, warp = tid >> 5;
+    if (tid == 0) s_base[0] = s_base[1] = 0;
+    for (int i0 = 0; i0 < b; i0 += kClassifyThreads) {
+        const int i = i0 + tid;
+        int tier = 0;
+        if (i < b) {
+            const int last = last_nodes[t0 + i];
+            if (last >= 0 && last < N) tier = node_tier[last];
+        }
+        const unsigned m1 = __ballot_sync(0xffffffffu, tier == 1), m2 = __ballot_sync(0xffffffffu, tier == 2);
+        __syncthreads();
+        if (lane == 0) {
+            s_w[0][warp] = __popc(m1);
+            s_w[1][warp] = __popc(m2);
+        }
+        __syncthreads();
+        int before1 = s_base[0], before2 = s_base[1];
+        for (int w = 0; w < warp; ++w) {
+            before1 += s_w[0][w];
+            before2 += s_w[1][w];
+        }
+        const unsigned lower = (1u << lane) - 1u;
+        if (tier == 1) list1[t0 + before1 + __popc(m1 & lower)] = t0 + i;
+        if (tier == 2) list2[t0 + before2 + __popc(m2 & lower)] = t0 + i;
+        __syncthreads();
+        if (tid == 0)
+            for (int w = 0; w < kClassifyThreads / 32; ++w) {
+                s_base[0] += s_w[0][w];
+                s_base[1] += s_w[1][w];
+            }
+    }
+    __syncthreads();
+    if (tid == 0) {
+        cnt1[t0] = s_base[0];
+        cnt2[t0] = s_base[1];
     }
 }
 
@@ -598,8 +649,16 @@
 void scone_table_destroy(FusedState* f) {
     cudaFree(f->d_cone_ptr); cudaFree(f->d_cone_ent); cudaFree(f->d_node_off); cudaFree(f->d_tb_rowptr); cudaFree(f->d_tb_ent);
     cudaFree(f->d_pair_ptr); cudaFree(f->d_tb_pairs); cudaFree(f->d_pair_off);
+    cudaFree(f->d_node_tier); cudaFree(f->d_tier_list); cudaFree(f->d_tier_cnt);
+    if (f->plan_side) cudaStreamDestroy(f->plan_side);
+    if (f->plan_tier0) cudaStreamDestroy(f->plan_tier0);
+    if (f->ev_plan_fork) cudaEventDestroy(f->ev_plan_fork);
+    if (f->ev_plan_join) cudaEventDestroy(f->ev_plan_join);
+    if (f->ev_plan_join0) cudaEventDestroy(f->ev_plan_join0);
     f->d_cone_ptr = nullptr; f->d_cone_ent = nullptr; f->d_node_off = nullptr; f->d_tb_rowptr = nullptr; f->d_tb_ent = nullptr;
     f->d_pair_ptr = nullptr; f->d_tb_pairs = nullptr; f->d_pair_off = nullptr;
+    f->d_node_tier = nullptr; f->d_tier_list = nullptr; f->d_tier_cnt = nullptr;
+    f->plan_side = nullptr; f->plan_tier0 = nullptr; f->ev_plan_fork = nullptr; f->ev_plan_join = nullptr; f->ev_plan_join0 = nullptr;
     f->tb_rows = false;
 }
 
@@ -615,22 +674,25 @@
     int* d_cnt_m = nullptr;
     unsigned* d_cnt_e = nullptr;
     int* d_cnt_p = nullptr;
+    int* d_cnt_n1 = nullptr;
+    SCONE_CUDA(cudaMalloc((void**)&d_cnt_n1, (size_t)N * sizeof(int)));
     SCONE_CUDA(cudaMalloc((void**)&d_cnt_m, (size_t)N * sizeof(int)));
     SCONE_CUDA(cudaMalloc((void**)&d_cnt_e, (size_t)N * sizeof(unsigned)));
     SCONE_CUDA(cudaMalloc((void**)&d_cnt_p, (size_t)N * sizeof(int)));
     BuildArgs a{};
     a.nbrhoods = cx->d_nbrhoods; a.inc_ptr = cx->d_inc_ptr; a.inc_ent = cx->d_inc_ent; a.mptr = cx->d_mptr; a.ment = cx->d_ment;
     a.N = N; a.D = D; a.L = L; a.stats = f->d_stats;
-    a.cnt_m = d_cnt_m; a.cnt_e = d_cnt_e; a.cnt_p = d_cnt_p;
+    a.cnt_m = d_cnt_m; a.cnt_e = d_cnt_e; a.cnt_p = d_cnt_p; a.cnt_n1 = d_cnt_n1;
     table_build_kernel<<<N, kTbThreads, smem>>>(a);
     SCONE_LAUNCHED();
-    std::vector<int> st(n_stats), cm((size_t)N), cp((size_t)N);
+    std::vector<int> st(n_stats), cm((size_t)N), cp((size_t)N), c1((size_t)N);
     std::vector<unsigned> ce((size_t)N);
     SCONE_CUDA(cudaMemcpy(st.data(), f->d_stats, n_stats * sizeof(int), cudaMemcpyDeviceToHost));
     SCONE_CUDA(cudaMemcpy(cm.data(), d_cnt_m, (size_t)N * sizeof(int), cudaMemcpyDeviceToHost));
     SCONE_CUDA(cudaMemcpy(ce.data(), d_cnt_e, (size_t)N * sizeof(unsigned), cudaMemcpyDeviceToHost));
     SCONE_CUDA(cudaMemcpy(cp.data(), d_cnt_p, (size_t)N * sizeof(int), cudaMemcpyDeviceToHost));
-    cudaFree(d_cnt_m); cudaFree(d_cnt_e); cudaFree(d_cnt_p);
+    SCONE_CUDA(cudaMemcpy(c1.data(), d_cnt_n1, (size_t)N * sizeof(int), cudaMemcpyDeviceToHost));
+    cudaFree(d_cnt_m); cudaFree(d_cnt_e); cudaFree(d_cnt_p); cudaFree(d_cnt_n1);
     std::vector<unsigned> cone_ptr((size_t)N + 1), pair_ptr((size_t)N + 1);
     std::vector<unsigned long long> node_off((size_t)N + 1);
     unsigned long long tm = 0, te = 0, tp = 0;
@@ -682,7 +744,7 @@
     SCONE_CUDA(cudaMalloc((void**)&f->d_cone_ptr, cone_ptr.size() * sizeof(unsigned)));
     SCONE_CUDA(cudaMalloc((void**)&f->d_cone_ent, (size_t)(tm ? tm : 1) * sizeof(uint32_t)));
     SCONE_CUDA(cudaMemcpy(f->d_cone_ptr, cone_ptr.data(), cone_ptr.size() * sizeof(unsigned), cudaMemcpyHostToDevice));
-    a.cnt_m = nullptr; a.cnt_e = nullptr; a.cnt_p = nullptr;
+    a.cnt_m = nullptr; a.cnt_e = nullptr; a.cnt_p = nullptr; a.cnt_n1 = nullptr;
     a.cone_ptr = f->d_cone_ptr; a.keys = f->d_cone_ent; a.with_rows = want_rows ? 1 : 0;
     if (want_rows) {
         SCONE_CUDA(cudaMalloc((void**)&f->d_node_off, node_off.size() * sizeof(unsigned long long)));
@@ -715,14 +777,38 @@
             const char* v = getenv(name);
             return v && *v ? atoi(v) : dflt;
         };
+        int q99_n1 = f->bound_list;
+        {
+            std::vector<int> s1(c1);
+            const size_t k99 = std::min(s1.size() - 1, (s1.size() * 99 + 99) / 100 - 1);
+            std::nth_element(s1.begin(), s1.begin() + k99, s1.end());
+            q99_n1 = std::max(1, s1[k99]);
+        }
         f->tbM0 = std::min(f->tbM, (env_int("SCONE_TABLE_M0", f->quantile_cone) + 63) & ~63);
-        f->tbLV0 = std::min(f->tbLV, (env_int("SCONE_TABLE_LV0", 192) + 63) & ~63);
+        f->tbLV0 = std::min(f->tbLV, (env_int("SCONE_TABLE_LV0", q99_n1) + 63) & ~63);
         f->tb_two_tiers = f->tbM0 < f->tbM || f->tbLV0 < f->tbLV;
         f->tb_smem0 = table_plan_smem(f->tbM0, f->tbLV0);
         f->tbM1 = std::min(f->tbM, (env_int("SCONE_TABLE_M1", std::max(quantile999, 2 * f->tbM0)) + 63) & ~63);
-        f->tbLV1 = std::min(f->tbLV, (env_int("SCONE_TABLE_LV1", 512) + 63) & ~63);
+        int lv1 = 1;
+        for (int n = 0; n < N; ++n)
+            if (cm[n] <= f->tbM1) lv1 = std::max(lv1, c1[n]);
+        f->tbLV1 = std::min(f->tbLV, (env_int("SCONE_TABLE_LV1", lv1) + 63) & ~63);
         f->tb_smem1 = table_plan_smem(f->tbM1, f->tbLV1);
-        f->tb_mid_tier = f->tb_two_tiers && (f->tbM1 > f->tbM0 || f->tbLV1 > f->tbLV0) && 2 * f->tb_smem1 <= f->tb_smem;
+        f->tb_mid_tier = f->tb_two_tiers && (f->tbM1 > f->tbM0 || f->tbLV1 > f->tbLV0) && (f->tbM1 < f->tbM || f->tbLV1 < f->tbLV);
+        if (f->tb_two_tiers) {
+            std::vector<uint8_t> tier((size_t)N);
+            for (int n = 0; n < N; ++n)
+                tier[n] = cm[n] <= f->tbM0 && c1[n] <= f->tbLV0 ? 0 : (f->tb_mid_tier && cm[n] <= f->tbM1 && c1[n] <= f->tbLV1 ? 1 : 2);
+            SCONE_CUDA(cudaMalloc((void**)&f->d_node_tier, (size_t)N));
+            SCONE_CUDA(cudaMemcpy(f->d_node_tier, tier.data(), (size_t)N, cudaMemcpyHostToDevice));
+            int prio_lo = 0, prio_hi = 0;
+            SCONE_CUDA(cudaDeviceGetStreamPriorityRange(&prio_lo, &prio_hi));
+            SCONE_CUDA(cudaStreamCreateWithPriority(&f->plan_side, cudaStreamNonBlocking, prio_hi));
+            SCONE_CUDA(cudaStreamCreateWithPriority(&f->plan_tier0, cudaStreamNonBlocking, prio_hi < prio_lo ? prio_hi + 1 : prio_hi));
+            SCONE_CUDA(cudaEventCreateWithFlags(&f->ev_plan_fork, cudaEventDisableTiming));
+            SCONE_CUDA(cudaEventCreateWithFlags(&f->ev_plan_join, cudaEventDisableTiming));
+            SCONE_CUDA(cudaEventCreateWithFlags(&f->ev_plan_join0, cudaEventDisableTiming));
+        }
         SCONE_CUDA(cudaFuncSetAttribute(table_plan_kernel<64>, cudaFuncAttributeMaxDynamicSharedMemorySize, (int)kMaxTablePlanSmem));
         SCONE_CUDA(cudaFuncSetAttribute(table_plan_kernel<128>, cudaFuncAttributeMaxDynamicSharedMemorySize, (int)kMaxTablePlanSmem));
         SCONE_CUDA(cudaFuncSetAttribute(table_plan_kernel<256>, cudaFuncAttributeMaxDynamicSharedMemorySize, (int)kMaxTablePlanSmem));
@@ -732,39 +818,60 @@
     return 0;
 }
 
-int scone_table_plan_launch(const FusedState* f, PlanArgs p, int b, int num_sms, cudaStream_t st, int phase) {
-    const int f_chunk = f->chunk;
+int scone_table_plan_launch(FusedState* f, PlanArgs p, int off, int b, int num_sms, cudaStream_t st) {
     p.cone_ptr = f->d_cone_ptr; p.cone_ent = f->d_cone_ent; p.node_off = f->d_node_off; p.tb_rowptr = f->d_tb_rowptr; p.tb_ent = f->d_tb_ent;
     p.pair_ptr = f->d_pair_ptr; p.tb_pairs = f->d_tb_pairs; p.pair_off = f->d_pair_off;
-    p.tier = 0; p.n_work = b;
-    p.M = f->tbM0; p.LV = f->tbLV0;
-    int* list0 = p.retry;
-    int* list1 = p.retry + f_chunk;
-    int* cnt0 = p.n_retry;
-    int* cnt1 = p.n_retry + 1;
-    p.retry = f->tb_two_tiers ? list0 : nullptr;
-    p.n_retry = cnt0;
-    if (phase != 1) {
-        static const int t0 = [] { const char* v = getenv("SCONE_TABLE_T0"); return v && *v ? atoi(v) : 128; }();
-        if (t0 == 64) table_plan_kernel<64><<<b, 64, f->tb_smem0, st>>>(p);
-        else if (t0 == 256) table_plan_kernel<256><<<b, 256, f->tb_smem0, st>>>(p);
-        else table_plan_kernel<128><<<b, 128, f->tb_smem0, st>>>(p);
+    p.retry = nullptr; p.n_retry = nullptr;
+    if (f->tb_two_tiers) {
+        SCONE_CUDA(cudaEventRecord(f->ev_plan_fork, st));
+        SCONE_CUDA(cudaStreamWaitEvent(f->plan_side, f->ev_plan_fork, 0));
+        SCONE_CUDA(cudaStreamWaitEvent(f->plan_tier0, f->ev_plan_fork, 0));
+        f->plan_forked = true;
+        int* list1 = f->d_tier_list;
+        int* list2 = f->d_tier_list + f->chunk;
+        int* cnt1 = f->d_tier_cnt;
+        int* cnt2 = f->d_tier_cnt + f->chunk;
+        table_classify_kernel<<<1, kClassifyThreads, 0, f->plan_side>>>(p.last_nodes, f->d_node_tier, p.N, off, b, list1, list2, cnt1, cnt2);
         SCONE_LAUNCHED();
-    }
-    if (!f->tb_two_tiers || phase == 0) return 0;
-    const int* n_in = cnt0;
-    const int* in_list = list0;
-    if (f->tb_mid_tier) {
-        p.tier = 1; p.M = f->tbM1; p.LV = f->tbLV1; p.n_in = n_in; p.in_list = in_list; p.retry = list1; p.n_retry = cnt1;
-        const int per_sm = std::max(1, std::min(8, (int)((size_t)220 * 1024 / (f->tb_smem1 + 1024))));
-        table_plan_kernel<256><<<std::min(b, per_sm * num_sms), 256, f->tb_smem1, st>>>(p);
+        if (f->tb_mid_tier) {
+            PlanArgs q = p;
+            q.tier = 1; q.M = f->tbM1; q.LV = f->tbLV1; q.n_in = cnt1 + off; q.in_list = list1 + off;
+            const int per_sm = std::max(1, std::min(8, (int)((size_t)220 * 1024 / (f->tb_smem1 + 1024))));
+            table_plan_kernel<256><<<std::min(b, per_sm * num_sms), 256, f->tb_smem1, f->plan_side>>>(q);
+            SCONE_LAUNCHED();
+        }
+        PlanArgs q = p;
+        q.tier = 2; q.M = f->tbM; q.LV = f->tbLV; q.n_in = cnt2 + off; q.in_list = list2 + off;
+        const int per_sm = std::max(1, std::min(4, (int)((size_t)220 * 1024 / (f->tb_smem + 1024))));
+        table_plan_kernel<kTier1Threads><<<std::min(b, per_sm * num_sms), kTier1Threads, f->tb_smem, f->plan_side>>>(q);
         SCONE_LAUNCHED();
-        n_in = cnt1;
-        in_list = list1;
-    }
-    p.tier = 2; p.M = f->tbM; p.LV = f->tbLV; p.n_in = n_in; p.in_list = in_list; p.retry = nullptr; p.n_retry = cnt0;
-    const int per_sm = std::max(1, std::min(4, (int)((size_t)220 * 1024 / (f->tb_smem + 1024))));
-    table_plan_kernel<512><<<std::min(b, per_sm * num_sms), 512, f->tb_smem, st>>>(p);
+    }
+    p.tier = 0; p.n_work = b; p.t0 = off; p.M = f->tbM0; p.LV = f->tbLV0;
+    p.node_tier = f->tb_two_tiers ? f->d_node_tier : nullptr;
+    const cudaStream_t s0 = f->tb_two_tiers ? f->plan_tier0 : st;
+    static const int t0 = [] { const char* v = getenv("SCONE_TABLE_T0"); return v && *v ? atoi(v) : 128; }();
+    if (t0 == 64) table_plan_kernel<64><<<b, 64, f->tb_smem0, s0>>>(p);
+    else if (t0 == 256) table_plan_kernel<256><<<b, 256, f->tb_smem0, s0>>>(p);
+    else table_plan_kernel<128><<<b, 128, f->tb_smem0, s0>>>(p);
     SCONE_LAUNCHED();
     return 0;
 }
+
+int scone_table_plan_join(FusedState* f, cudaStream_t st) {
+    if (!f->plan_forked) return 0;
+    SCONE_CUDA(cudaEventRecord(f->ev_plan_join, f->plan_side));
+    SCONE_CUDA(cudaEventRecord(f->ev_plan_join0, f->plan_tier0));
+    SCONE_CUDA(cudaStreamWaitEvent(st, f->ev_plan_join, 0));
+    SCONE_CUDA(cudaStreamWaitEvent(st, f->ev_plan_join0, 0));
+    f->plan_forked = false;
+    return 0;
+}
+
+int scone_fused_node_tiers(const FusedState* f, int N, uint8_t* out) {
+    if (f->d_node_tier == nullptr) {
+        memset(out, 0, (size_t)N);
+        return 0;
+    }
+    SCONE_CUDA(cudaMemcpy(out, f->d_node_tier, (size_t)N, cudaMemcpyDeviceToHost));
+    return 0;
+}
diff --git a/scone_gcn_b200/model.py b/scone_gcn_b200/model.py
--- a/scone_gcn_b200/model.py
+++ b/scone_gcn_b200/model.py
@@ -46,6 +46,12 @@
                 'live_rows_tier0', 'plan_smem_tier0_kb', 'two_tiers', 'table_plan_mb', 'arena_mwords', 'cone_table_kentries', 'retries_last_chunk']
         return dict(zip(keys, (int(v) for v in out)))
 
+    def fused_node_tiers(self):
+        out = np.zeros(self.cx.N, np.uint8)
+        sizes = np.zeros(6, np.int32)
+        _lib.check(_lib.lib().scone_model_fused_node_tiers(self.handle, _lib.ptr(out), _lib.ptr(sizes)), 'scone_model_fused_node_tiers')
+        return out, dict(zip(['M0', 'LV0', 'M1', 'LV1', 'M', 'LV'], (int(v) for v in sizes)))
+
     def fused_header(self, t):
         hdr = np.zeros(16, np.int32)
         _lib.check(_lib.lib().scone_model_fused_read(self.handle, int(t), _lib.ptr(hdr), 0, 0, None), 'scone_model_fused_read')
```

Measured after the change: 7.430 million, median of 6. No clear change (-0.2%).
